# linchaobao/EPPM

Measured on AMD Instinct MI355X. Metric: Mflow-vectors/sec, higher is better.
Workload: dtype f32; 1 GPU; single 1024x436 Sintel-shape synthetic pair per step, full 3-level pyramid, patch_r=9, default defs.h parameters; 1 rank(s), independent pairs; inputs: RGBA planes resident in HBM before the timed region; outputs: interleaved float2 flow left in HBM (the PCIe-inclusive window of the reference API -- host RGB in, host u/v out -- is `host_boundary`, with --full); inputs=device-resident RGBA, outputs=device-resident float2 flow, pairs_in_flight_per_gpu=24, pairs_per_launch=8, contexts_in_flight=3, width=1024, height=436

## Files before the change

eppm_amd/_lib.py:

```python
import ctypes as C
import os

from .build import lib_path


class EppmError(RuntimeError):
    pass


class CParams(C.Structure):
    _fields_ = [("patch_r", C.c_int), ("num_iter", C.c_int), ("search_range", C.c_int), ("num_guess", C.c_int),
                ("seg_len", C.c_int), ("wmf_iters", C.c_int), ("seed", C.c_ulonglong), ("propagation", C.c_int),
                ("levels", C.c_int)]


class CTrackParams(C.Structure):
    _fields_ = [("spacing", C.c_int), ("min_eig", C.c_int64), ("fb_alpha", C.c_float), ("fb_beta", C.c_float), ("mb_alpha", C.c_float),
                ("mb_beta", C.c_float), ("capacity", C.c_int)]


class CTFilterParams(C.Structure):
    _fields_ = [("thresh", C.c_float), ("n_max", C.c_int)]


# ... 50 lines not shown

    def as_dict(self):
        return {k: int(getattr(self, k)) for k, _ in self._fields_}


class CObject(C.Structure):
    _fields_ = [("id", C.c_int32), ("age", C.c_int32), ("area", C.c_int32), ("x0", C.c_int32), ("y0", C.c_int32), ("x1", C.c_int32),
                ("y1", C.c_int32), ("n_flow", C.c_int32), ("sum_x", C.c_int64), ("sum_y", C.c_int64), ("sum_qu", C.c_int64), ("sum_qv", C.c_int64)]

    def as_dict(self):
        return {k: int(getattr(self, k)) for k, _ in self._fields_}


class CObjectsCounts(C.Structure):
    _fields_ = [("n", C.c_int32), ("n_found", C.c_int32), ("n_components", C.c_int32), ("next_id", C.c_int32)]

    def as_dict(self):
        return {k: int(getattr(self, k)) for k, _ in self._fields_}


class CTrackCounts(C.Structure):
    _fields_ = [("live", C.c_int), ("ended", C.c_int), ("seeded", C.c_int), ("dropped", C.c_int), ("frame", C.c_int), ("next_id", C.c_int)]

    def as_dict(self):
        return {k: int(getattr(self, k)) for k, _ in self._fields_}


_lib = None

SYMBOLS = [
    "eppm_default_params", "eppm_create", "eppm_create_batch", "eppm_batch_size", "eppm_batch_set_images", "eppm_batch_set_images_device",
    "eppm_batch_compute", "eppm_batch_compute_device", "eppm_batch_compute_end", "eppm_batch_get_plane", "eppm_destroy", "eppm_set_stream", "eppm_set_images", "eppm_set_images_device",
    "eppm_compute", "eppm_compute_begin", "eppm_compute_end", "eppm_compute_device", "eppm_synchronize", "eppm_num_levels", "eppm_level_dims", "eppm_get_plane",
    "eppm_stage_times", "eppm_clear_stage_times", "eppm_enable_stage_timing", "eppm_last_error", "eppm_version",
    "eppm_device_count", "eppm_set_device", "eppm_malloc_device", "eppm_malloc_pitched", "eppm_free_device",
    "eppm_memcpy_h2d", "eppm_memcpy_d2h", "eppm_memcpy2d_h2d", "eppm_memcpy2d_d2h", "eppm_memset_device",
    "eppm_device_synchronize", "eppm_device_mem_info", "eppm_device_pci_bus_id", "eppm_bind_thread_to_device", "eppm_release_cached_memory", "eppm_set_launcher_stream", "eppm_set_launcher_params", "eppm_launcher_status",
    "baoCudaPatchMatchMultiscalePrepare", "baoCudaCensusTransform", "baoCudaPatchMatch", "baoCudaLeftRightCheck",
    "baoCudaOutlierRemoval", "baoCudaWeightedMedianFilter", "baoCudaFillHole", "baoCudaNNF2Flow", "baoCudaBLF_C2F",
    "baoCudaBLFCostFilterRefine", "baoCudaFlowSmoothing", "eppm_flow_to_color", "eppm_compute_color",
    "eppm_pm_rng_create", "eppm_pm_rng_reset", "eppm_pm_rng_destroy", "eppm_pm_rng_block_states", "eppm_pm_gen_rand_field",
    "eppm_pm_cost_field", "eppm_pm_seg_propagate", "eppm_pm_jump_propagate", "eppm_pm_parallel_propagate", "eppm_pm_random_search", "eppm_gauss_filter_rgba", "eppm_resize_rgba",
    "eppm_resize_flow",
    "eppm_host_register", "eppm_host_unregister", "eppm_host_is_registered", "eppm_host_alloc", "eppm_host_free",
    "eppm_compute_begin_into", "eppm_batch_compute_begin_into",
    "eppm_load_ppm", "eppm_ppm_size", "eppm_save_flo", "eppm_load_flo", "eppm_flo_size", "eppm_flow_error",
    "eppm_flow_error_border", "eppm_flow_error_percentage", "eppm_flow_cutoff", "eppm_flow_to_color_host",
    "eppm_compute_bidirectional", "eppm_compute_bidirectional_device", "eppm_batch_compute_bidirectional", "eppm_set_occlusion_params",
    "eppm_fb_occlusion", "eppm_fb_occlusion_host",
    "eppm_interpolate", "eppm_interpolate_device", "eppm_batch_interpolate", "eppm_interpolate_frames", "eppm_interpolate_host",
    "eppm_track_default_params", "eppm_track_capacity", "eppm_tracker_create", "eppm_tracker_destroy", "eppm_track_step",
    "eppm_track_step_frames", "eppm_tracker_get", "eppm_tracker_get_ended", "eppm_tracker_set", "eppm_track_step_host", "eppm_track_seeds_host",
    "eppm_push_image", "eppm_push_image_device", "eppm_set_temporal", "eppm_temporal_reset", "eppm_temporal_valid", "eppm_temporal_prior_host",
    "eppm_temporal_prior",
    "eppm_batch_set_temporal", "eppm_batch_push_images", "eppm_batch_push_images_device", "eppm_batch_temporal_valid", "eppm_batch_temporal_reset",
    "eppm_temporal_prior_batch",
    "eppm_set_stop_level", "eppm_stop_level", "eppm_flow_upsample",
    "eppm_tfilter_default_params", "eppm_tfilter_create", "eppm_tfilter_create_size", "eppm_tfilter_destroy", "eppm_tfilter_reset", "eppm_tfilter_step",
    "eppm_tfilter_step_frames", "eppm_tfilter_get", "eppm_tfilter_get_device", "eppm_tfilter_get_state", "eppm_tfilter_set_state",
    "eppm_tfilter_seed_host", "eppm_tfilter_step_host",
    "eppm_stab_default_params", "eppm_stab_create", "eppm_stab_create_size", "eppm_stab_destroy", "eppm_stab_reset", "eppm_stab_step",
    "eppm_stab_step_frames", "eppm_stab_get", "eppm_stab_get_device", "eppm_stab_get_mask", "eppm_stab_get_model", "eppm_stab_get_path",
    "eppm_stab_set_path", "eppm_gmotion_fit_host", "eppm_stab_update_host", "eppm_stab_warp_host",
    "eppm_cutdet_default_params", "eppm_cutdet_create", "eppm_cutdet_create_size", "eppm_cutdet_destroy", "eppm_cutdet_step",
    "eppm_cutdet_step_frames", "eppm_cutdet_get", "eppm_cutdet_cuts", "eppm_cutdet_host",
    "eppm_mblur_default_params", "eppm_motion_blur", "eppm_motion_blur_device", "eppm_batch_motion_blur", "eppm_motion_blur_frames",
    "eppm_motion_blur_host",
    "eppm_cmap_default_params", "eppm_cmap_create", "eppm_cmap_create_size", "eppm_cmap_destroy", "eppm_cmap_reset", "eppm_cmap_step",
    "eppm_cmap_step_frames", "eppm_cmap_get_state", "eppm_cmap_set_state", "eppm_cmap_set_layer", "eppm_cmap_render", "eppm_cmap_render_device",
    "eppm_cmap_age", "eppm_cmap_step_host", "eppm_cmap_render_host",
    "eppm_objects_default_params", "eppm_objects_create", "eppm_objects_create_size", "eppm_objects_destroy", "eppm_objects_reset",
    "eppm_objects_step", "eppm_objects_step_frames", "eppm_objects_get", "eppm_objects_get_labels", "eppm_objects_get_state",
    "eppm_objects_set_state", "eppm_objects_label_host", "eppm_objects_carry_host", "eppm_objects_assign_host",
    "eppm_plate_default_params", "eppm_plate_create", "eppm_plate_create_size", "eppm_plate_destroy", "eppm_plate_reset", "eppm_plate_canvas_dims",
    "eppm_plate_step", "eppm_plate_step_frames", "eppm_plate_render", "eppm_plate_render_frames", "eppm_plate_get", "eppm_plate_get_device",
    "eppm_plate_get_mask", "eppm_plate_get_path", "eppm_plate_set_path", "eppm_plate_get_state", "eppm_plate_set_state",
    "eppm_plate_forms_host", "eppm_plate_block_host", "eppm_plate_accumulate_host", "eppm_plate_render_host",
    "eppm_defect_default_params", "eppm_defect_create", "eppm_defect_create_size", "eppm_defect_destroy", "eppm_defect_reset", "eppm_defect_step",
    "eppm_defect_step_frames", "eppm_defect_get", "eppm_defect_get_device", "eppm_defect_get_mask", "eppm_defect_get_stats",
    "eppm_defect_get_state", "eppm_defect_set_state", "eppm_defect_step_host",
]


TEST_SYMBOLS = ["eppm_test_set_option", "eppm_test_c2f_refine_batch", "eppm_probe_c2f_window", "eppm_probe_dispatch", "eppm_probe_fast_exp", "eppm_probe_div_const", "eppm_probe_delta_table",
                "eppm_probe_unpack_texel", "eppm_probe_pm_parity", "eppm_probe_ctx_rng_states", "eppm_test_pm_search", "eppm_probe_search_pretest", "eppm_probe_launch_log"]

_variant = None


def select_library(variant):
    global _variant
    if _lib is not None and variant != _variant:
        raise EppmError("select_library: a library is loaded already")
    _variant = variant


def lib():
    global _lib
    if _lib is None:
        path = lib_path(_variant)
        if not os.path.exists(path):
            raise EppmError(f"{path} is missing: run eppm_amd.build() (hipcc --offload-arch=gfx950); there is no CPU fallback")
        L = C.CDLL(path)
        L.eppm_last_error.restype = C.c_char_p
        L.eppm_version.restype = C.c_char_p
        _plate_signatures(L)
        _lib = L
    return _lib


def _plate_signatures(L):
    P, I, Z, F = C.c_void_p, C.c_int, C.c_size_t, C.c_float
    sig = {
        "eppm_plate_default_params": [P], "eppm_plate_create": [P, P, P], "eppm_plate_create_size": [I, I, I, I, P, P], "eppm_plate_destroy": [P],
        "eppm_plate_reset": [P, I], "eppm_plate_canvas_dims": [P, P, P], "eppm_plate_step": [P, P, P],
        "eppm_plate_step_frames": [P, I, P, Z, P, P, I], "eppm_plate_render": [P, P, I, P, Z, P],
        "eppm_plate_render_frames": [P, I, P, Z, P, P, P, Z, P], "eppm_plate_get": [P, I, P, Z, P], "eppm_plate_get_device": [P, I, P, Z],
        "eppm_plate_get_mask": [P, I, P], "eppm_plate_get_path": [P, I, P], "eppm_plate_set_path": [P, I, P], "eppm_plate_get_state": [P, I, P],
        "eppm_plate_set_state": [P, I, P], "eppm_plate_forms_host": [P, P, P, P], "eppm_plate_block_host": [P, P, I, I, P],
        "eppm_plate_accumulate_host": [P, P, P, P, I, I, P], "eppm_plate_render_host": [P, P, I, P, P, I, I, P, P, P],
    }
    for name, args in sig.items():
        fn = getattr(L, name, None)
        if fn is None:
            continue
        fn.argtypes = args
        fn.restype = I


def check(status, what=""):
    if status != 0:
        raise EppmError(f"{what}: status {status}: {lib().eppm_last_error().decode()}")


def check_launcher(what=""):
    check(lib().eppm_launcher_status(), what)


LAUNCH_STAGES = ("smoothing", "jbu", "refine", "search", "sweep", "sweeps_merged")


class launch_log:

    def __enter__(self):
        check(lib().eppm_test_set_option(b"launch_log", 1), "launch_log on")
        self._kept = None
        return self

    def entries(self):
        if self._kept is not None:
            return self._kept
        n = lib().eppm_probe_launch_log(None, 0)
        buf = (C.c_int * (6 * max(n, 1)))()
        n = min(n, lib().eppm_probe_launch_log(buf, n))
        return [(LAUNCH_STAGES[buf[6 * i]],) + tuple(buf[6 * i + 1:6 * i + 6]) for i in range(n)]

    def __exit__(self, *exc):
        self._kept = self.entries()
        lib().eppm_test_set_option(b"launch_log", 0)
        return False


def probe_dispatch(stage, *args, nout=1):
    a = (C.c_int * len(args))(*[int(v) for v in args])
    out = (C.c_int * nout)()
    check(lib().eppm_probe_dispatch(stage.encode(), a, len(args), out, nout), f"eppm_probe_dispatch {stage}")
    return tuple(out)
# ... 1 lines not shown
```

eppm_amd/csrc/api_internal.h:

```cpp
#pragma once

#include <ctype.h>
#include <math.h>
#include <sched.h>
#include <stdarg.h>
#include <stdio.h>
#include <stdlib.h>
#include <string.h>

#include <atomic>
#include <chrono>
#include <condition_variable>
#include <map>
#include <mutex>
#include <string>
#include <tuple>
#include <vector>

#include "eppm_internal.h"
#include "host_registry.h"

#define EPPM_HIDDEN __attribute__((visibility("hidden")))

EPPM_HIDDEN int set_err(int code, const char* fmt, ...) __attribute__((format(printf, 2, 3)));
#define HIPCHK(expr)                                                                                         \
    do {                                                                                                     \
        hipError_t e_ = (expr);                                                                              \
        if (e_ != hipSuccess) {                                                                              \
            (void)hipGetLastError();                                                                         \
            return set_err(EPPM_ERR_HIP, "%s failed: %s (%s:%d)", #expr, hipGetErrorString(e_), __FILE__, __LINE__); \
        }                                                                                                    \
    } while (0)
#define CHK(expr)                     \
    do {                              \
        int r_ = (expr);              \
        if (r_ != EPPM_OK) return r_; \
    } while (0)

EPPM_HIDDEN int check_params(const eppm_params& p);
EPPM_HIDDEN void host_pm_lut(int R, std::vector<float>& v);
EPPM_HIDDEN void host_wmf_lut(std::vector<float>& v);
EPPM_HIDDEN void host_blf_lut(std::vector<float>& v);
EPPM_HIDDEN int pyr_init_dim(int* arrH, int* arrW, int h, int w, int maxDepth, double ratio);
EPPM_HIDDEN int upload_lut(float** dst, const std::vector<float>& v);
struct DeltaIndex { int32_t t1[256]; std::vector<float> dval; };
EPPM_HIDDEN const DeltaIndex& delta_index();
EPPM_HIDDEN int upload_lut_delta(float** dst, const std::vector<float>& head, int which);
EPPM_HIDDEN int upload_pm_lut(float** dst, int R);
EPPM_HIDDEN int upload_wmf_lut(float** dst);
EPPM_HIDDEN int upload_blf_lut(float** dst);

#ifdef EPPM_TEST_HOOKS
EPPM_HIDDEN extern std::atomic<int> g_opt_rand_table;
EPPM_HIDDEN extern std::atomic<int> g_opt_sweep_spec;
EPPM_HIDDEN extern std::atomic<int> g_opt_no_split;
EPPM_HIDDEN extern std::atomic<int> g_opt_force_split;
EPPM_HIDDEN extern std::atomic<int> g_opt_search_pre;
static inline int opt_rand_table() { return g_opt_rand_table.load(); }
static inline int opt_sweep_spec() { return g_opt_sweep_spec.load(); }
static inline int opt_no_split() { return g_opt_no_split.load(); }
static inline int opt_force_split() { return g_opt_force_split.load(); }
static inline int opt_search_pre() { return g_opt_search_pre.load(); }
EPPM_HIDDEN extern std::atomic<int> g_opt_alloc_fill;
static inline int opt_alloc_fill() { return g_opt_alloc_fill.load(); }
EPPM_HIDDEN hipError_t alloc_fill(hipError_t e, void* p, size_t bytes, bool pinned);
#else
static constexpr int opt_rand_table() { return 1; }
static constexpr int opt_sweep_spec() { return -1; }
static constexpr int opt_no_split() { return 0; }
static constexpr int opt_force_split() { return 0; }
static constexpr int opt_search_pre() { return -1; }
static constexpr int opt_alloc_fill() { return -1; }
#endif


namespace eppm { struct RngTables; }
struct eppm_pm_rng {
    eppm::RngTables* tables = nullptr;
    const int16_t* rand_tab = nullptr;
    size_t rand_stride = 0;
    int device = 0, w = 0, h = 0, gx = 0, gy = 0, G = 0, per_lane = 0;
    unsigned long long seed = 0;
    uint32_t* init_tab = nullptr;
    uint32_t* iter_tab = nullptr;
    uint32_t* work[2][2] = {{nullptr, nullptr}, {nullptr, nullptr}};
    bool own_work = true;
    int cur[2] = {0, 0};
    uint32_t* skip_mat = nullptr;
    uint32_t skip_weyl = 0;
    eppm::PmRngDev dev() const
    {
        eppm::PmRngDev d;
        d.init_tab = init_tab; d.iter_tab = iter_tab; d.skip_mat = skip_mat;
        d.skip_weyl = skip_weyl; d.per_lane = per_lane; d.gx = gx; d.gy = gy;
        return d;
    }
};
EPPM_HIDDEN int rng_create(eppm_pm_rng** out, int w, int h, const eppm_params& p, bool alloc_work = true);
EPPM_HIDDEN void rng_free(eppm_pm_rng* r);
EPPM_HIDDEN void rngtab_release_idle();

EPPM_HIDDEN hipError_t cache_alloc(void** p, size_t bytes, bool pinned, int device);
EPPM_HIDDEN void cache_free(void* p, size_t bytes, bool pinned, int device);
EPPM_HIDDEN hipError_t pooled_stream_create(hipStream_t* out, int device);
EPPM_HIDDEN void pooled_stream_destroy(hipStream_t s, int device);

EPPM_HIDDEN eppm::PmProblem mk_problem(const eppm::PlanesH& P, float* cost, int16_t* nnf, int16_t* nnf_alt, eppm_pm_rng* rng, int k, float* spec = nullptr,
                                       int32_t* scand = nullptr, uint32_t* wl = nullptr, int16_t* seed = nullptr, float* restw = nullptr);
EPPM_HIDDEN void search(eppm::PmBatch& b, eppm_pm_rng* rng, const float* lut, const eppm_params& prm, hipStream_t s, int launch_no = -1, bool pretest = false);
EPPM_HIDDEN bool sweep_list_on(int mode);
EPPM_DECISION bool sweep_speculative(int iteration, long long pixels, int m);
EPPM_DECISION bool sweeps_merged(int iteration, long long pixels, long long problem_pixels, int m);
EPPM_HIDDEN void sweep(eppm::PmBatch& b, const float* lut, const eppm_params& prm, int dir, hipStream_t s, bool speculative = false);
EPPM_HIDDEN void jump(eppm::PmBatch& b, const float* lut, const eppm_params& prm, hipStream_t s);
EPPM_HIDDEN void neighbor(eppm::PmBatch& b, const float* lut, const eppm_params& prm, int launches, hipStream_t s);
EPPM_HIDDEN void run_patchmatch(eppm::PmBatch& b, eppm_pm_rng* rng, const float* lut, const eppm_params& prm, hipStream_t s, int spec_mode, int pre_from = -1);
EPPM_HIDDEN void pm_start(eppm::PmBatch& b, eppm_pm_rng* rng, const float* lut, const eppm_params& prm, hipStream_t s, int pre_from = -1);
EPPM_HIDDEN void pm_iterate(eppm::PmBatch& b, eppm_pm_rng* rng, const float* lut, const eppm_params& prm, hipStream_t s, int spec_mode, int pre_from = -1);
#ifndef EPPM_SWEEP_CACHE
#define EPPM_SWEEP_CACHE 1
#endif

EPPM_HIDDEN int launcher_finish();

EPPM_HIDDEN int ctx_device(const eppm_ctx* c, int* h, int* w);
EPPM_HIDDEN void ctx_stage_begin(eppm_ctx* c, const char* name);
EPPM_HIDDEN void ctx_stage_end(eppm_ctx* c);

EPPM_HIDDEN int stab_step_on(eppm_stab* f, eppm::StabArgs& in, int slot0, const uint8_t* cut, hipStream_t s, eppm_ctx* timing);
EPPM_HIDDEN const uint8_t* stab_mask_device(const eppm_stab* f, size_t* slot_stride);
EPPM_HIDDEN const char* stab_model_device(const eppm_stab* f, size_t* slot_stride);
```

eppm_amd/csrc/c2f_device.cuh:

```cuda
#pragma once
#include "eppm_device.cuh"

#ifndef EPPM_C2F_UNROLL
#define EPPM_C2F_UNROLL 2
#endif
#ifndef EPPM_C2F_WAVES
#define EPPM_C2F_WAVES 4
#endif
#ifndef EPPM_C2F_WAVES_MIN
#define EPPM_C2F_WAVES_MIN 2
#endif
#define EPPM_C2F_OCC __attribute__((amdgpu_waves_per_eu(EPPM_C2F_WAVES_MIN, EPPM_C2F_WAVES)))
#ifndef EPPM_C2F_WIN_H
#ifdef EPPM_TOL
#define EPPM_C2F_WIN_H 50
#else
#define EPPM_C2F_WIN_H 48
#endif
#endif
#ifndef EPPM_C2F_PASS2
#define EPPM_C2F_PASS2 1
#endif
#ifndef EPPM_C2F_WIN_WAVES
#define EPPM_C2F_WIN_WAVES 4
#endif
#ifndef EPPM_C2F_SPLIT_BELOW_WAVES
#define EPPM_C2F_SPLIT_BELOW_WAVES 1024
#endif
#ifndef EPPM_C2F_WINDOW
#define EPPM_C2F_WINDOW 1
#endif
#ifndef EPPM_C2F_WINDOW17
#define EPPM_C2F_WINDOW17 1
#endif
#ifdef EPPM_TOL
#define EPPM_C2F_LOG2 true
#else
#define EPPM_C2F_LOG2 false
#endif
#define EPPM_PRAGMA_(x) _Pragma(#x)
#define EPPM_UNROLL(n) EPPM_PRAGMA_(unroll n)

namespace eppm {

__device__ __forceinline__ Planes to_dev(const PlanesH& h, size_t pstride = 0, unsigned pair = 0)
{
    Planes p;
    p.pk1 = pair_ptr((const float4*)h.pk1, pstride, pair); p.pk2 = pair_ptr((const float4*)h.pk2, pstride, pair);
    p.w = h.w; p.h = h.h; p.pitch = h.pitch;
    return p;
}

__device__ __forceinline__ float4 stage_texel(const uint32_t* __restrict__ pc, const float4* __restrict__ pk, unsigned idx)
{
    if (pc) { const uint32_t w = pc[idx]; return make_texel(w, w >> 24); }
    return pk[idx];
}

__device__ __forceinline__ bool c2f_unknown(float fvx, float fvy) { return fvx > kUnknownFlowThresh || fvy > kUnknownFlowThresh; }
__device__ __forceinline__ int c2f_centre(float f, int x) { return (int)(int16_t)(f2short(f) + x); }
__device__ __forceinline__ void c2f_store_flow(float* flow, int idx, int fx, int fy)
{
    flow[idx * 2] = (float)fx;
    flow[idx * 2 + 1] = (float)fy;
}
__device__ __forceinline__ float c2f_min(float a, float b) { return (a < b) ? a : b; }
__device__ __forceinline__ float c2f_min4(float c1, float c2, float c3, float c4) { return c2f_min(c1, c2f_min(c2, c2f_min(c3, c4))); }
template <class F>
__device__ __forceinline__ void c2f_select_best(float* flow, int x, int y, int ccx, int ccy, int w, int h, F cost_of)
{
    int bx = ccx, by = ccy;
    float min_cost = 999999;
#pragma unroll
    for (int m = 0; m < 3; m++) {
        const int cx = (int)(int16_t)(ccx + m - 1);
        if (cx < 0 || cx >= w) continue;
#pragma unroll
        for (int n = 0; n < 3; n++) {
            const int cy = (int)(int16_t)(ccy + n - 1);
            if (cy < 0 || cy >= h) continue;
            const float cv = cost_of(m, n);
            if (cv < min_cost) { min_cost = cv; bx = cx; by = cy; }
        }
    }
    flow[(y * w + x) * 2] = (float)(bx - x);
    flow[(y * w + x) * 2 + 1] = (float)(by - y);
}

template <int SPLIT>
__device__ __forceinline__ bool c2f_tile_origin(const Planes& P, int& x0, int& y0, int& part)
{
    const int tiles_x = (P.w + kBlock - 1) / kBlock, tiles = tiles_x * ((P.h + kBlock - 1) / kBlock);
    const int per_xcd = (tiles + 7) / 8;
    const int slot = SPLIT ? (blockIdx.x >> 3) / SPLIT : (blockIdx.x >> 3);
    part = SPLIT ? (blockIdx.x >> 3) % SPLIT : -1;
    const int tile = (blockIdx.x & 7) * per_xcd + slot;
    if (slot >= per_xcd || tile >= tiles) return false;
    x0 = (tile % tiles_x) * kBlock; y0 = (tile / tiles_x) * kBlock;
    return true;
}

template <int R> struct C2fSrcTile { static constexpr int TWU = kBlock + 2 * R, TW = (TWU + 15) / 16 * 16; };
struct C2fOff { int dx16, up; };

template <int R>
struct C2fTables {
    static constexpr int S = R + 1;
    C2fOff off[3][S * S];
    int rowdy[3][S];
};

constexpr int cfloor(float v) { const int t = (int)v; return ((float)t > v) ? t - 1 : t; }
template <int R>
constexpr C2fTables<R> make_c2f_tables()
{
    constexpr int S = R + 1;
    constexpr float kc[3][4] = {
        {0.177f, -0.011f, -0.003f, 0.301f},
        {0.125f, -0.357f, 0.009f, 0.308f},
        {0.205f, 0.370f, 0.011f, 0.296f},
    };
    C2fTables<R> T{};
    for (int p = 0; p < 3; p++)
        for (int ii = 0; ii < S; ii++) {
            const int i = 2 * ii - R;
            int dy[S] = {};
            int lo = 1 << 30;
            for (int jj = 0; jj < S; jj++) {
                const int j = 2 * jj - R;
                const float fx = (float)(j)*kc[p][0] + (float)(i)*kc[p][1];
                const float fy = (float)(j)*kc[p][2] + (float)(i)*kc[p][3];
                T.off[p][ii * S + jj].dx16 = (j + cfloor(fx)) * 16;
                dy[jj] = i + cfloor(fy);
                lo = dy[jj] < lo ? dy[jj] : lo;
            }
            T.rowdy[p][ii] = lo;
            for (int jj = 0; jj < S; jj++) T.off[p][ii * S + jj].up = dy[jj] - lo;
        }
    return T;
}
template <int R> __device__ __forceinline__ const C2fTables<R>& c2f_tables();

template <int R>
struct C2fWinShape {
    static constexpr int xlo() { int v = -R; const auto T = make_c2f_tables<R>(); for (int p = 0; p < 3; p++) for (int t = 0; t < (R + 1) * (R + 1); t++) v = T.off[p][t].dx16 / 16 < v ? T.off[p][t].dx16 / 16 : v; return v; }
    static constexpr int xhi() { int v = R; const auto T = make_c2f_tables<R>(); for (int p = 0; p < 3; p++) for (int t = 0; t < (R + 1) * (R + 1); t++) v = T.off[p][t].dx16 / 16 > v ? T.off[p][t].dx16 / 16 : v; return v; }
    static constexpr int ylo() { int v = -R; const auto T = make_c2f_tables<R>(); for (int p = 0; p < 3; p++) for (int i = 0; i <= R; i++) v = T.rowdy[p][i] < v ? T.rowdy[p][i] : v; return v; }
    static constexpr int yhi() { int v = R; const auto T = make_c2f_tables<R>(); for (int p = 0; p < 3; p++) for (int i = 0; i <= R; i++) v = T.rowdy[p][i] + 1 > v ? T.rowdy[p][i] + 1 : v; return v; }
    static constexpr int XLO = xlo(), XHI = xhi(), YLO = ylo(), YHI = yhi();
    static constexpr int WW = (R == 9) ? 64 : (kBlock + 2 + (XHI - XLO) + 8 + 15) / 16 * 16;
    static constexpr int WH = (R == 9) ? EPPM_C2F_WIN_H : kBlock + 2 + (YHI - YLO) + 7;
    static constexpr int SPAN_X = WW - 3 - (XHI - XLO), SPAN_Y = WH - 3 - (YHI - YLO);
    static_assert(SPAN_X >= kBlock - 1 && SPAN_Y >= kBlock - 1, "window too small for a constant-flow tile (spread kBlock - 1)");
};

#ifdef EPPM_TOL
struct C2fSample { rgbf p1; uint32_t k1; float lsrc; };
__device__ __forceinline__ rgbf c2f_weight_centre(const rgbf c) { return tol_scale_centre(c); }
template <class LUT>
__device__ __forceinline__ C2fSample c2f_sample(const LUT& L, const rgbf c1, const float4 q1, int t)
{
    const rgbf p1 = texel_rgb(q1);
    const uint32_t k1 = __float_as_uint(q1.w);
    return {p1, k1, tol_exp_arg_scaled(c1, p1, L.gsp[t])};
}
template <class LUT>
__device__ __forceinline__ void c2f_term(const LUT& L, const C2fSample& s, const rgbf c2, const float4 q2, float& cs, float& ws)
{
    const rgbf p2 = texel_rgb(q2);
    const float cost = tol_cost(L.tab(), s.p1, p2, s.k1, __float_as_uint(q2.w));
    patch_accum(cs, ws, cost, __builtin_amdgcn_exp2f(tol_exp_arg_scaled(c2, p2, s.lsrc)));
}
#else
struct C2fSample { rgbf p1; uint32_t k1; float a2, gsp; };
__device__ __forceinline__ rgbf c2f_weight_centre(const rgbf c) { return c; }
template <class LUT>
__device__ __forceinline__ C2fSample c2f_sample(const LUT& L, const rgbf c1, const float4 q1, int t)
{
    const rgbf p1 = texel_rgb(q1);
    const uint32_t k1 = __float_as_uint(q1.w);
    float a2 = max_abs_diff(c1, p1);
    a2 *= a2;
    return {p1, k1, a2, L.gsp[t]};
}
template <class LUT>
// ... 71 lines not shown
template <int R, int PASS, bool RAW = false, bool WIN = false, int WW = 0>
__device__ __forceinline__ void c2f_pass(const Planes& P, const PatchLutT<R + 1>& L, const float4* __restrict__ s_src,
                                         int TW, int tx, int ty, int cx16, int wmax16, int ccy, const rgbf c1, const rgbf (&c2)[3], float (&run)[3],
                                         const float4* __restrict__ s_win = nullptr, int wbase = 0)
{
    constexpr int S = R + 1;
    constexpr int TP = (PASS == 0) ? 0 : PASS - 1;
    const C2fTables<R>& T = c2f_tables<R>();
    const rgbf c1w = c2f_weight_centre(c1), c2w[3] = {c2f_weight_centre(c2[0]), c2f_weight_centre(c2[1]), c2f_weight_centre(c2[2])};
    float cs[3] = {0.0f, 0.0f, 0.0f}, ws[3] = {0.0f, 0.0f, 0.0f};
    const unsigned pitch16 = (unsigned)P.pitch << 4;
#pragma unroll 1
    for (int ii = 0; ii < S; ii++) {
        unsigned Rr[4];
        const int rdy = (PASS == 0) ? 2 * ii - R : T.rowdy[TP][ii];
        const int rb = ccy - 1 + rdy;
        if (!WIN) {
#pragma unroll
            for (int k = 0; k < 4; k++) Rr[k] = __umul24((unsigned)iclamp(rb + k, 0, P.h - 1), pitch16);
        }
EPPM_UNROLL(EPPM_C2F_UNROLL)
        for (int jj = 0; jj < S; jj++) {
            const C2fSample smp = c2f_sample(L, c1w, s_src[(ty + 2 * ii) * TW + tx + 2 * jj], ii * S + jj);
            const int dx16 = (PASS == 0) ? (2 * jj - R) * 16 : T.off[TP][ii * S + jj].dx16;
            float4 q2[3];
            if (WIN) {
                const int soff = (rdy + ((PASS != 0) ? T.off[TP][ii * S + jj].up : 0)) * (WW * 16) + dx16;
                const char* wp = reinterpret_cast<const char*>(s_win) + (wbase + soff);
#pragma unroll
                for (int n = 0; n < 3; n++) q2[n] = *reinterpret_cast<const float4*>(wp + n * (WW * 16));
            } else {
                const unsigned Xb = (unsigned)med3i(cx16 + dx16, 0, wmax16);
                if (PASS != 0 && T.off[TP][ii * S + jj].up) {
#pragma unroll
                    for (int n = 0; n < 3; n++) q2[n] = texel_at(P.pk2, Rr[n + 1] + Xb);
                } else {
#pragma unroll
                    for (int n = 0; n < 3; n++) q2[n] = texel_at(P.pk2, Rr[n] + Xb);
                }
            }
#pragma unroll
            for (int n = 0; n < 3; n++) c2f_term(L, smp, c2w[n], q2[n], cs[n], ws[n]);
        }
    }
#pragma unroll
    for (int n = 0; n < 3; n++) {
        const float c = cs[n] / ws[n];
        run[n] = (RAW || PASS == 3) ? c : c2f_min(c, run[n]);
    }
}

template <int R, int PA, int PB, int WW>
__device__ __forceinline__ void c2f_pass2_win(const PatchLutT<R + 1>& L, const float4* __restrict__ s_src, int TW, int tx, int ty,
                                              const rgbf c1, const rgbf (&c2)[3], const float4* __restrict__ s_win, int wbase,
                                              float (&outA)[3], float (&outB)[3])
{
    constexpr int S = R + 1;
    constexpr int TA = (PA == 0) ? 0 : PA - 1, TB = (PB == 0) ? 0 : PB - 1;
    const C2fTables<R>& T = c2f_tables<R>();
    const rgbf c1w = c2f_weight_centre(c1), c2w[3] = {c2f_weight_centre(c2[0]), c2f_weight_centre(c2[1]), c2f_weight_centre(c2[2])};
    const rgbf c2w6[6] = {c2w[0], c2w[1], c2w[2], c2w[0], c2w[1], c2w[2]};
    float cs[6] = {0.0f, 0.0f, 0.0f, 0.0f, 0.0f, 0.0f}, ws[6] = {0.0f, 0.0f, 0.0f, 0.0f, 0.0f, 0.0f};
#pragma unroll 1
    for (int ii = 0; ii < S; ii++) {
        const int rdyA = (PA == 0) ? 2 * ii - R : T.rowdy[TA][ii];
        const int rdyB = (PB == 0) ? 2 * ii - R : T.rowdy[TB][ii];
EPPM_UNROLL(EPPM_C2F_UNROLL)
        for (int jj = 0; jj < S; jj++) {
            const C2fSample smp = c2f_sample(L, c1w, s_src[(ty + 2 * ii) * TW + tx + 2 * jj], ii * S + jj);
            const int soffA = (rdyA + ((PA != 0) ? T.off[TA][ii * S + jj].up : 0)) * (WW * 16) + ((PA == 0) ? (2 * jj - R) * 16 : T.off[TA][ii * S + jj].dx16);
            const int soffB = (rdyB + ((PB != 0) ? T.off[TB][ii * S + jj].up : 0)) * (WW * 16) + ((PB == 0) ? (2 * jj - R) * 16 : T.off[TB][ii * S + jj].dx16);
            const char* wa = reinterpret_cast<const char*>(s_win) + (wbase + soffA);
            const char* wb = reinterpret_cast<const char*>(s_win) + (wbase + soffB);
            float4 q[6];
#pragma unroll
            for (int n = 0; n < 3; n++) { q[n] = *reinterpret_cast<const float4*>(wa + n * (WW * 16)); q[3 + n] = *reinterpret_cast<const float4*>(wb + n * (WW * 16)); }
            c2f_terms<6>(L, smp, c2w6, q, cs, ws);
        }
    }
#pragma unroll
    for (int n = 0; n < 3; n++) { outA[n] = cs[n] / ws[n]; outB[n] = cs[3 + n] / ws[3 + n]; }
}

}
```

eppm_amd/csrc/context.cpp:

```cpp
#include "context.h"

using namespace eppm;

extern "C" int eppm_destroy(eppm_ctx* c)
{
    if (!c) return EPPM_OK;
    (void)hipSetDevice(c->device);
    if (c->stream) (void)hipStreamSynchronize(c->stream);
    c->out_hold.release();
    clear_events(c, c->ev);
    clear_events(c, c->ev_prep);
    for (hipEvent_t e : c->ev_pool) (void)hipEventDestroy(e);
    cache_free(c->slab, c->slab_bytes, false, c->device);
    if (c->h_color) (void)hipHostFree(c->h_color);
    for (int q = 0; q < 2; q++) {
        cache_free(c->h_rgb[q], c->h_rgb_bytes, true, c->device);
        if (c->ev_rgb[q]) (void)hipEventDestroy(c->ev_rgb[q]);
    }
    if (c->ev_h2d) (void)hipEventDestroy(c->ev_h2d);
    cache_free(c->h_flow, c->h_flow_bytes, true, c->device);
    cache_free(c->bwd, c->bwd_bytes, false, c->device);
    cache_free(c->h_bwd, c->h_bwd_bytes, true, c->device);
    cache_free(c->itp, c->itp_bytes, false, c->device);
    cache_free(c->h_itp, c->h_itp_bytes, true, c->device);
// ... 11 lines not shown
    struct Entry { int device, R; float *pm, *wmf, *blf; };
    static std::mutex mu;
    static std::vector<Entry> tab;
    std::lock_guard<std::mutex> lk(mu);
    for (const Entry& e : tab)
        if (e.device == device && e.R == R) { *pm = e.pm; *wmf = e.wmf; *blf = e.blf; return EPPM_OK; }
    Entry e{device, R, nullptr, nullptr, nullptr};
    CHK(upload_pm_lut(&e.pm, R));
    CHK(upload_wmf_lut(&e.wmf));
    CHK(upload_blf_lut(&e.blf));
    tab.push_back(e);
    *pm = e.pm; *wmf = e.wmf; *blf = e.blf;
    return EPPM_OK;
}

static int ctx_alloc(eppm_ctx* c)
{
    const int h = c->h, w = c->w;
    Carve cv;
    auto pitch_of = [](size_t row_bytes) { return (row_bytes + 255) & ~(size_t)255; };
    c->raw_pitch = pitch_of((size_t)w * 4);
    for (uint32_t** p : {&c->raw1, &c->raw2}) cv.plane(p, c->raw_pitch * h);
    for (int i = 0; i < c->nl; i++) {
        c->ipitch[i] = pitch_of((size_t)c->W[i] * 4);
        c->cpitch[i] = pitch_of((size_t)c->W[i]);
        const size_t n = (size_t)c->W[i] * c->H[i];
        for (uint32_t** p : {&c->img1[i], &c->img2[i], &c->tmpu[i]}) cv.plane(p, c->ipitch[i] * c->H[i]);
        for (void** p : {&c->pk1[i], &c->pk2[i]}) cv.plane(p, n * 16);
        for (uint32_t** p : {&c->pc1[i], &c->pc2[i]}) cv.plane(p, n * 4);
        for (uint8_t** p : {&c->cen1[i], &c->cen2[i]}) cv.plane(p, c->cpitch[i] * c->H[i]);
        for (float** p : {&c->flow[i], &c->flow_tmp[i]}) cv.plane(p, n * 8);
        if (i < c->nl - 1 && c2f_refine_wants_split(c->W[i], c->H[i], c->prm.patch_r, 1, c->opt_no_split != 0)) cv.plane(&c->c2f_cost9[i], n * 36 * 4);
    }
    const int L = c->nl - 1;
    const size_t n2 = (size_t)c->W[L] * c->H[L];
#ifndef EPPM_TOL
    if (c->prm.patch_r == 9)
#endif
    {
        c->pp_pad = (c->prm.patch_r + 2) & ~1;
        c->pp_pitch = parity_pitch(c->W[L], c->pp_pad);
        for (uint32_t** p : {&c->pp1, &c->pp2}) cv.plane(p, (size_t)2 * c->H[L] * c->pp_pitch * 4);
    }
    for (int16_t** p : {&c->nnf1, &c->nnf2, &c->nnf_tmp, &c->nnf_tmp2}) cv.plane(p, n2 * 4);
    for (float** p : {&c->cost1, &c->cost2}) cv.plane(p, n2 * 4);
    for (float** p : {&c->spec1, &c->spec2}) cv.plane(p, n2 * 4 * 4);
    if (pm_search_pretest_form(c->W[L], c->H[L], c->prm.patch_r, 2, c->npairs))
        for (float** p : {&c->restw1, &c->restw2}) cv.plane(p, n2 * 4);
    for (int32_t** p : {&c->scand1, &c->scand2}) cv.plane(p, n2 * 4 * 4);
    for (uint32_t** p : {&c->wl1, &c->wl2}) cv.plane(p, pm_worklist_words(c->W[L], c->H[L], c->prm.seg_len) * 4);
    for (int16_t** p : {&c->seed1, &c->seed2}) cv.plane(p, n2 * 4 * 4);
    cv.plane(&c->wmf_ws, wmf_workspace_words(c->W[L], c->H[L], c->prm.wmf_iters) * 4);
    cv.plane(&c->d_rgb, (size_t)h * w * 3 * 2);
    cv.plane(&c->d_color, (size_t)h * w * 4);
    cv.plane(&c->d_uv, (size_t)h * w * 8);
    CHK(rng_create(&c->rng, c->W[L], c->H[L], c->prm, false));
    const size_t rng_bytes = (size_t)c->rng->gx * c->rng->gy * 64 * 6 * 4;
    for (int k = 0; k < 2; k++)
        for (int q = 0; q < 2; q++) cv.plane(&c->rng->work[k][q], rng_bytes);
    c->stride = (cv.off + 4095) & ~(size_t)4095;
    CHK(cv.alloc(&c->slab, &c->slab_bytes, c->stride * c->npairs, c->device, (std::to_string(c->npairs) + " slab(s)").c_str()));
    CHK(shared_luts(c->device, c->prm.patch_r, &c->lut_pm, &c->lut_wmf, &c->lut_blf));
    c->out_u.assign(c->npairs, nullptr);
    c->out_v.assign(c->npairs, nullptr);
    for (auto* v : {&c->tmp_snap, &c->tmp_valid, &c->tmp_seeded, &c->tmp_cut}) v->assign(c->npairs, 0);
    return EPPM_OK;
}

extern "C" int eppm_create_batch(eppm_ctx** out, int h, int w, int device, const eppm_params* params, int npairs)
{
    if (!out) return set_err(EPPM_ERR_ARG, "eppm_create: NULL out");
    *out = nullptr;
    if (npairs < 1 || npairs > 4096) return set_err(EPPM_ERR_ARG, "eppm_create_batch: npairs %d out of range [1,4096]", npairs);
    if (h < 4 || w < 4 || h > 32767 || w > 32767) return set_err(EPPM_ERR_ARG, "eppm_create: size %dx%d out of range (NNF coordinates are int16)", w, h);
    if ((unsigned long long)h * (unsigned long long)w * 16ULL >= (1ULL << 32))
        return set_err(EPPM_ERR_ARG, "eppm_create: size %dx%d out of range (texel planes are addressed with 32-bit byte offsets)", w, h);
    eppm_params p;
    eppm_default_params(&p);
    if (params) p = *params;
    CHK(check_params(p));
    HIPCHK(hipSetDevice(device));
    eppm_ctx* c = new eppm_ctx();
    c->device = device; c->prm = p; c->h = h; c->w = w; c->npairs = npairs; c->n_active = 1;
    c->opt_sweep_spec = opt_sweep_spec(); c->opt_no_split = opt_no_split(); c->opt_search_pre = opt_search_pre();
    c->nl = pyr_init_dim(c->H, c->W, h, w, p.levels, 0.5f);
    const int L = c->nl - 1;
    if (c->H[L] < 1 || c->W[L] < 1 || (c->W[L] + p.seg_len - 1) / p.seg_len > 1024 || (c->H[L] + p.seg_len - 1) / p.seg_len > 1024) {
        delete c;
        return set_err(EPPM_ERR_ARG, "eppm_create: unsupported size %dx%d", w, h);
    }
    const hipError_t e = pooled_stream_create(&c->stream, c->device);
    if (e != hipSuccess) { delete c; return set_err(EPPM_ERR_HIP, "hipStreamCreate: %s", hipGetErrorString(e)); }
    c->own_stream = true;
    int r = ctx_alloc(c);
    if (r != EPPM_OK) { eppm_destroy(c); return r; }
    *out = c;
    return EPPM_OK;
}

extern "C" int eppm_create(eppm_ctx** out, int h, int w, int device, const eppm_params* params)
{
    return eppm_create_batch(out, h, w, device, params, 1);
}

extern "C" int eppm_batch_size(const eppm_ctx* c) { return c ? c->npairs : 0; }

extern "C" int eppm_set_stream(eppm_ctx* c, void* s)
{
    if (!c) return set_err(EPPM_ERR_ARG, "NULL ctx");
    if (c->own_stream && c->stream) { (void)hipStreamSynchronize(c->stream); pooled_stream_destroy(c->stream, c->device); }
    c->stream = (hipStream_t)s;
    c->own_stream = false;
    return EPPM_OK;
}

extern "C" int eppm_num_levels(const eppm_ctx* c) { return c ? c->nl : 0; }
extern "C" int eppm_level_dims(const eppm_ctx* c, int level, int* h, int* w)
{
    if (!c || level < 0 || level >= c->nl) return set_err(EPPM_ERR_ARG, "bad level");
    if (h) *h = c->H[level];
    if (w) *w = c->W[level];
    return EPPM_OK;
}
extern "C" int eppm_enable_stage_timing(eppm_ctx* c, int on)
{
    if (!c) return set_err(EPPM_ERR_ARG, "NULL ctx");
    c->timing = (on == 2) ? 2 : (on != 0);
    return EPPM_OK;
}

int ctx_device(const eppm_ctx* c, int* h, int* w)
{
    *h = c->h;
    *w = c->w;
    return c->device;
}

void ctx_stage_begin(eppm_ctx* c, const char* name) { stage_begin(c, c->ev, name); }
void ctx_stage_end(eppm_ctx* c) { stage_end(c, c->ev); }

extern "C" int eppm_synchronize(eppm_ctx* c)
{
    if (!c) return set_err(EPPM_ERR_ARG, "NULL ctx");
    HIPCHK(hipStreamSynchronize(c->stream));
    return EPPM_OK;
}

extern "C" int eppm_stage_times(eppm_ctx* c, const char** names, float* ms, int max)
{
    if (!c) return 0;
    (void)hipStreamSynchronize(c->stream);
    int n = 0;
    for (auto* v : {&c->ev_prep, &c->ev})
        for (auto& e : *v) {
            if (n >= max) return n;
            float t = 0;
            if (hipEventElapsedTime(&t, e.a, e.b) != hipSuccess) t = -1;
            names[n] = e.name; ms[n] = t; n++;
        }
    return n;
}

extern "C" int eppm_clear_stage_times(eppm_ctx* c)
{
    if (!c) return set_err(EPPM_ERR_ARG, "NULL ctx");
    (void)hipStreamSynchronize(c->stream);
    clear_events(c, c->ev);
// ... 86 lines not shown
```

eppm_amd/csrc/context.h:

```cpp
#pragma once

#include <algorithm>

#include "api_internal.h"

struct StageEv { const char* name; hipEvent_t a, b; };

struct eppm_ctx {
    int device = 0;
    hipStream_t stream = nullptr;
    bool own_stream = false;
    int opt_sweep_spec = -1, opt_no_split = 0, opt_search_pre = -1;
    eppm_params prm;
    int h = 0, w = 0, nl = 0;
    int stop_level = 0;
    int npairs = 1, n_active = 1;
    char* slab = nullptr;
    size_t stride = 0;
    int H[eppm::kMaxLevels], W[eppm::kMaxLevels];
    size_t ipitch[eppm::kMaxLevels], cpitch[eppm::kMaxLevels];
    uint32_t *raw1 = nullptr, *raw2 = nullptr;
    size_t raw_pitch = 0;
    uint32_t *img1[eppm::kMaxLevels] = {}, *img2[eppm::kMaxLevels] = {}, *tmpu[eppm::kMaxLevels] = {};
    uint8_t *cen1[eppm::kMaxLevels] = {}, *cen2[eppm::kMaxLevels] = {};
    void *pk1[eppm::kMaxLevels] = {}, *pk2[eppm::kMaxLevels] = {};
    uint32_t *pc1[eppm::kMaxLevels] = {}, *pc2[eppm::kMaxLevels] = {};
    uint32_t *pp1 = nullptr, *pp2 = nullptr;
    int pp_pitch = 0, pp_pad = 0;
    int16_t *nnf1 = nullptr, *nnf2 = nullptr, *nnf_tmp = nullptr, *nnf_tmp2 = nullptr;
    float *cost1 = nullptr, *cost2 = nullptr;
    float *spec1 = nullptr, *spec2 = nullptr;
    int32_t *scand1 = nullptr, *scand2 = nullptr;
    uint32_t *wl1 = nullptr, *wl2 = nullptr;
    float *restw1 = nullptr, *restw2 = nullptr;
    int16_t *seed1 = nullptr, *seed2 = nullptr;
    uint32_t* wmf_ws = nullptr;
    bool flow_pending = false;
    float *flow[eppm::kMaxLevels] = {}, *flow_tmp[eppm::kMaxLevels] = {};
    float* c2f_cost9[eppm::kMaxLevels] = {};
    float *lut_pm = nullptr, *lut_wmf = nullptr, *lut_blf = nullptr;
    eppm_pm_rng* rng = nullptr;
    float* d_uv = nullptr;
    uint32_t* d_color = nullptr;
    uint32_t* h_color = nullptr;
    uint8_t* d_rgb = nullptr;
    size_t slab_bytes = 0, h_rgb_bytes = 0, h_flow_bytes = 0;
    uint8_t* h_rgb[2] = {nullptr, nullptr};
    hipEvent_t ev_rgb[2] = {nullptr, nullptr};
    hipEvent_t ev_h2d = nullptr;
    int rgb_cur = 0;
    float* h_flow = nullptr;
    std::vector<float*> out_u, out_v;
    eppm::HostHold out_hold;
    bool have_images = false, have_flow = false;
    char* bwd = nullptr;
    size_t bwd_stride = 0, bwd_bytes = 0, h_bwd_bytes = 0;
    float* bflow[eppm::kMaxLevels] = {};
    float* d_buv = nullptr;
    uint8_t *occ1 = nullptr, *occ2 = nullptr;
    uint8_t* h_bwd = nullptr;
    float occ_alpha = 0.01f, occ_beta = 0.5f;
    bool have_bwd = false;
    bool bwd_images = false;
    char* itp = nullptr;
    size_t itp_bytes = 0, itp_plane = 0, h_itp_bytes = 0;
    uint64_t* itp_keys = nullptr;
    int32_t *itp_fill1 = nullptr, *itp_fill2 = nullptr;
    uint8_t* itp_rgb = nullptr;
    uint8_t* h_itp = nullptr;
    char* mbl = nullptr;
    size_t mbl_bytes = 0, mbl_plane = 0, mbl_tplane = 0, h_mbl_bytes = 0;
    uint32_t* mbl_packed = nullptr;
    uint64_t* mbl_tkeys = nullptr;
    uint8_t* mbl_rgb = nullptr;
    uint8_t* h_mbl = nullptr;
    bool temporal = false;
    std::vector<uint8_t> tmp_snap;
    std::vector<uint8_t> tmp_valid;
    std::vector<uint8_t> tmp_seeded;
    std::vector<uint8_t> tmp_cut;
    char* tmp = nullptr;
    size_t tmp_bytes = 0, tmp_stride = 0;
    int16_t *prev_fwd = nullptr, *prev_bwd = nullptr, *prior1 = nullptr, *prior2 = nullptr, *nnf_init1 = nullptr, *nnf_init2 = nullptr;
    float *cost_init1 = nullptr, *cost_init2 = nullptr;
    int32_t* tmp_keys = nullptr;
    void tmp_drop() { std::fill(tmp_valid.begin(), tmp_valid.end(), 0); std::fill(tmp_snap.begin(), tmp_snap.end(), 0); std::fill(tmp_cut.begin(), tmp_cut.end(), 0); }
    int timing = 0;
    std::vector<StageEv> ev;
    std::vector<StageEv> ev_prep;
    std::vector<hipEvent_t> ev_pool;
    eppm::Batch bt() const { return eppm::Batch{n_active, stride}; }
    template <class T> T* of_pair(T* p, int k) const { return (T*)((char*)p + (size_t)k * stride); }
    template <class T> T* of_bwd_pair(T* p, int k) const { return (T*)((char*)p + (size_t)k * bwd_stride); }
};

// ... 83 lines not shown
```

eppm_amd/csrc/ctx_compute.cpp:

```cpp
#include "context.h"
#include "temporal.h"

using namespace eppm;

static int tmp_alloc(eppm_ctx* c)
{
    if (c->tmp) return EPPM_OK;
    const int L = c->nl - 1;
    const size_t n2 = (size_t)c->W[L] * c->H[L];
    Carve cv;
    for (int16_t** p : {&c->prev_fwd, &c->prev_bwd, &c->prior1, &c->prior2, &c->nnf_init1, &c->nnf_init2}) cv.plane(p, n2 * 4);
    for (float** p : {&c->cost_init1, &c->cost_init2}) cv.plane(p, n2 * 4);
    cv.plane(&c->tmp_keys, n2 * 4 * 2);
    c->tmp_stride = cv.off;
    CHK(cv.alloc(&c->tmp, &c->tmp_bytes, c->tmp_stride * c->npairs, c->device, "temporal planes"));
    for (int k = 0; k < c->npairs; k++) launch_temporal_keys_init((int32_t*)((char*)c->tmp_keys + (size_t)k * c->tmp_stride), (int)(2 * n2), c->stream);
    HIPCHK(hipGetLastError());
    return EPPM_OK;
}

static int set_temporal(eppm_ctx* c, int on)
{
    c->temporal = on != 0;
    if (!on) c->tmp_drop();
// ... 7 lines not shown
}
extern "C" int eppm_temporal_reset(eppm_ctx* c)
{
    if (!c) return set_err(EPPM_ERR_ARG, "eppm_temporal_reset: NULL ctx");
    return eppm_batch_temporal_reset(c, 0);
}
extern "C" int eppm_temporal_valid(const eppm_ctx* c) { return eppm_batch_temporal_valid(c, 0); }

extern "C" int eppm_batch_set_temporal(eppm_ctx* c, int on)
{
    if (!c) return set_err(EPPM_ERR_ARG, "eppm_batch_set_temporal: NULL ctx");
    return set_temporal(c, on);
}
extern "C" int eppm_batch_temporal_reset(eppm_ctx* c, int pair)
{
    if (!c) return set_err(EPPM_ERR_ARG, "eppm_batch_temporal_reset: NULL ctx");
    if (pair >= c->npairs) return set_err(EPPM_ERR_ARG, "eppm_batch_temporal_reset: pair %d, context holds %d", pair, c->npairs);
    for (int k = pair < 0 ? 0 : pair; k < (pair < 0 ? c->npairs : pair + 1); k++) c->tmp_valid[k] = c->tmp_snap[k] = 0;
    return EPPM_OK;
}
extern "C" int eppm_batch_temporal_valid(const eppm_ctx* c, int pair)
{
    return c && pair >= 0 && pair < c->npairs && c->temporal && c->tmp_valid[pair] ? 1 : 0;
}

struct Branch {
    int16_t *&nnf, *&nnf_alt;
    float* cost;
    uint32_t* const* guide;
    bool swap, bwd, dominant;
    int16_t* snapshot;
    float *a[kMaxLevels], *b[kMaxLevels];
};

enum { kStageUp, kStageRefine, kStageBlf, kStageJbu };
static const struct EPPM_HIDDEN LevelStageNames {
    char s[4][2][kMaxLevels][24];
    LevelStageNames()
    {
        const char* base[4] = {"upsample", "c2f_refine", "flow_blf", "flow_jbu"};
        for (int k = 0; k < 4; k++)
            for (int b = 0; b < 2; b++)
                for (int l = 0; l < kMaxLevels; l++) snprintf(s[k][b][l], sizeof s[k][b][l], "%s%s_L%d", base[k], b ? "_bwd" : "", l);
    }
} level_stage;

static void branch_nnf2flow(eppm_ctx* c, Branch& d)
{
    hipStream_t s = c->stream;
    const Batch bt = c->bt();
    const int L = c->nl - 1, lw = c->W[L], lh = c->H[L], gp = (int)(c->ipitch[L] / 4);
    launch_outlier(d.nnf_alt, d.cost, d.nnf, lw, lh, lw, lw, s, bt);
    std::swap(d.nnf, d.nnf_alt);
    if (launch_wmf(d.nnf, d.nnf_alt, d.guide[L], gp, lw, lh, lw, c->lut_wmf, c->prm.wmf_iters, 1, c->wmf_ws, s, bt) != d.nnf)
        std::swap(d.nnf, d.nnf_alt);
    launch_fill_holes(d.nnf_alt, d.nnf, d.guide[L], gp, lw, lh, lw, s, bt);
    std::swap(d.nnf, d.nnf_alt);
    if (d.snapshot) launch_nnf2flow_snapshot(d.a[L], lw, d.snapshot, c->tmp_stride, d.nnf, lw, lw, lh, s, bt);
    else launch_nnf2flow(d.a[L], lw, d.nnf, lw, lw, lh, s, bt);
}

static int branch_c2f(eppm_ctx* c, Branch& d, int (*keep)(eppm_ctx*, int, float*))
{
    hipStream_t s = c->stream;
    const Batch bt = c->bt();
    const int L = c->nl - 1;
    auto blf = [&](float* dst, const float* src, int l) { launch_flow_blf(dst, src, d.guide[l], (int)(c->ipitch[l] / 4), c->W[l], c->H[l], c->W[l], c->lut_blf, s, bt); };
    const int stop = c->stop_level;
    float* r = d.a[L];
    for (int l = L - 1; l >= 0; l--) {
        if (l < stop) {
            stage_begin(c, c->ev, level_stage.s[kStageJbu][d.bwd][l]);
            float* out = (r == d.b[l]) ? d.a[l] : d.b[l];
            launch_flow_jbu(out, r, d.guide[l], (int)(c->ipitch[l] / 4), c->W[l], c->H[l], c->W[l + 1], c->H[l + 1], c->lut_blf, s, bt);
            r = out;
            CHK(keep(c, l, r));
            stage_end(c, c->ev);
            continue;
        }
        stage_begin(c, c->ev, level_stage.s[kStageUp][d.bwd][l]);
        launch_resize_flow(d.a[l], c->H[l], c->W[l], r, c->H[l + 1], c->W[l + 1], 2.0f, 2.0f, s, bt);
        stage_end(c, c->ev);
        stage_begin(c, c->ev, level_stage.s[kStageRefine][d.bwd][l], d.dominant);
        launch_c2f_refine(planes(c, l, d.swap), d.a[l], c->lut_pm, c->prm.patch_r, c->c2f_cost9[l], s, bt, c->opt_no_split != 0);
        stage_end(c, c->ev, d.dominant);
        stage_begin(c, c->ev, level_stage.s[kStageBlf][d.bwd][l]);
        blf(d.b[l], d.a[l], l);
        r = d.b[l];
        if (l > 0) CHK(keep(c, l, r));
        stage_end(c, c->ev);
    }
    if (stop > 0) return EPPM_OK;
    stage_begin(c, c->ev, d.bwd ? "flow_blf_bwd_final" : "flow_blf_final");
    float* out = (r == d.b[0]) ? d.a[0] : d.b[0];
    blf(out, r, 0);
    CHK(keep(c, 0, out));
    stage_end(c, c->ev);
    return EPPM_OK;
}

static int keep_fwd(eppm_ctx* c, int l, float* r)
{
    if (r != c->flow[l]) std::swap(c->flow[l], c->flow_tmp[l]);
    return EPPM_OK;
}

static int compute_all(eppm_ctx* c)
{
    if (!c->have_images) return set_err(EPPM_ERR_STATE, "eppm_compute: no images set");
    HIPCHK(hipSetDevice(c->device));
    c->have_bwd = false;
    hipStream_t s = c->stream;
    const Batch bt = c->bt();
    const int L = c->nl - 1, lw = c->W[L], lh = c->H[L];

    const bool tmode = c->temporal;
    bool seeded = false;
    std::fill(c->tmp_seeded.begin(), c->tmp_seeded.end(), 0);
    if (tmode) {
        CHK(tmp_alloc(c));
        TemporalArgs a{};
        for (int k = 0; k < bt.n; k++)
            if (c->tmp_valid[k]) { a.armed[k >> 5] |= 1u << (k & 31); seeded = true; }
        if (seeded) {
            a.prev[0] = c->prev_fwd; a.prior[0] = c->prior1; a.keys[0] = c->tmp_keys; a.step[0] = 1;
            a.prev[1] = c->prev_bwd; a.prior[1] = c->prior2; a.keys[1] = c->tmp_keys + (size_t)lw * lh; a.step[1] = -1;
            a.w = lw; a.h = lh; a.ndir = 2; a.nslots = bt.n; a.stride = c->tmp_stride;
            stage_begin(c, c->ev, "temporal_advect");
            launch_temporal_splat(a, s);
            launch_temporal_gather(a, s);
            stage_end(c, c->ev);
        }
    }
    std::fill(c->tmp_snap.begin(), c->tmp_snap.end(), 0);

    const size_t pm_entry = c->ev.size();
    stage_begin(c, c->ev, "patchmatch");
    {
        PmBatch b;
        b.n = 2; b.cpitch = lw; b.npitch = lw; b.npairs = bt.n; b.stride = bt.stride;
        b.cache_plane = (size_t)lw * lh;
        b.seed_plane = (size_t)lw * lh * 2;
        b.wl_units = pm_worklist_units(lw, lh, c->prm.seg_len);
        b.p[0] = mk_problem(planes(c, L, false), c->cost1, c->nnf1, c->nnf_tmp, c->rng, 0, c->spec1, EPPM_SWEEP_CACHE ? c->scand1 : nullptr, sweep_list_on(c->opt_sweep_spec) ? c->wl1 : nullptr, c->seed1, c->restw1);
        b.p[1] = mk_problem(planes(c, L, true), c->cost2, c->nnf2, c->nnf_tmp2, c->rng, 1, c->spec2, EPPM_SWEEP_CACHE ? c->scand2 : nullptr, sweep_list_on(c->opt_sweep_spec) ? c->wl2 : nullptr, c->seed2, c->restw2);
        if (!seeded) run_patchmatch(b, c->rng, c->lut_pm, c->prm, s, c->opt_sweep_spec, c->opt_search_pre);
        else {
            pm_start(b, c->rng, c->lut_pm, c->prm, s, c->opt_search_pre);
            PmSeed sd;
            sd.prior[0] = c->prior1; sd.nnf_init[0] = c->nnf_init1; sd.cost_init[0] = c->cost_init1;
            sd.prior[1] = c->prior2; sd.nnf_init[1] = c->nnf_init2; sd.cost_init[1] = c->cost_init2;
            sd.stride = c->tmp_stride;
            stage_begin(c, c->ev, "temporal_select");
            launch_pm_cost_select(b, sd, c->lut_pm, c->prm.patch_r, s);
            stage_end(c, c->ev);
            pm_iterate(b, c->rng, c->lut_pm, c->prm, s, c->opt_sweep_spec, c->opt_search_pre);
        }
    }
    stage_end_at(c, c->ev, pm_entry);
    if (tmode) launch_temporal_snapshot(c->prev_bwd, c->tmp_stride, c->nnf2, lw, lw, lh, s, bt);

    stage_begin(c, c->ev, "l2_post");
    launch_lr_check(c->nnf1, c->cost1, c->nnf2, lw, lh, lw, lw, s, bt);
    launch_lr_check(c->nnf2, c->cost2, c->nnf1, lw, lh, lw, lw, s, bt);
    Branch d{c->nnf1, c->nnf_tmp, c->cost1, c->img1, false, false, true, tmode ? c->prev_fwd : nullptr};
    for (int l = 0; l <= L; l++) { d.a[l] = c->flow[l]; d.b[l] = c->flow_tmp[l]; }
    branch_nnf2flow(c, d);
// ... 251 lines not shown
```

eppm_amd/csrc/eppm_device.cuh:

```cuda
#pragma once

#include <hip/hip_runtime.h>
#include <stdint.h>
#include <float.h>
#include <type_traits>

#include "eppm_internal.h"

namespace eppm {

template <class T>
__device__ __forceinline__ T* pair_ptr(T* p, size_t stride, unsigned pair)
{
    using Byte = typename std::conditional<std::is_const<T>::value, const char, char>::type;
    return reinterpret_cast<T*>(reinterpret_cast<Byte*>(p) + stride * pair);
}
template <class T>
__device__ __forceinline__ T* pair_ptr_opt(T* p, size_t stride, unsigned pair)
{
    return p ? pair_ptr(p, stride, pair) : p;
}

constexpr float kLambdaAd2 = 0.1f * 0.1f;
constexpr float kPmSigR2 = 0.1f * 0.1f;
// ... 50 lines not shown
    int r;
    asm("v_med3_i32 %0, %1, %2, %3" : "=v"(r) : "v"(v), "v"(lo), "v"(hi));
    return r;
}

__device__ __forceinline__ float max_abs_diff(const rgbf a, const rgbf b)
{
    return fmaxf(fmaxf(fabsf(a.x - b.x), fabsf(a.y - b.y)), fabsf(a.z - b.z));
}

struct Planes {
    const float4* pk1;
    const float4* pk2;
    int w, h;
    int pitch;
};

typedef uint32_t u32x4 __attribute__((ext_vector_type(4)));
typedef uint32_t u32x2 __attribute__((ext_vector_type(2)));

#ifndef EPPM_TOL
#ifndef EPPM_CENSUS_POPCNT
#define EPPM_CENSUS_POPCNT 1
#endif
__device__ __forceinline__ float4 make_texel(uint32_t rgba, uint32_t census)
{
    const rgbf c = unpack_rgb(rgba);
    return make_float4(c.x, c.y, c.z, __uint_as_float(EPPM_CENSUS_POPCNT ? (census & 0xffu) * 0x01010101u : (census & 0xffu) << 2));
}
__device__ __forceinline__ float census_cost(const float* __restrict__ cnx, uint32_t w1, uint32_t w2)
{
    return *reinterpret_cast<const float*>(reinterpret_cast<const char*>(cnx) + (EPPM_CENSUS_POPCNT ? (uint32_t)__builtin_popcount(w1 ^ w2) : (w1 ^ w2)));
}
__device__ __forceinline__ float4 unpack_texel(uint32_t w, uint32_t)
{
    static_assert(EPPM_CENSUS_POPCNT, "the census byte replicated into its word (make_texel)");
    const rgbf c = unpack_rgb(w);
    return make_float4(c.x, c.y, c.z, __uint_as_float(__builtin_amdgcn_perm(w, w, 0x03030303u)));
}
#else
constexpr unsigned kTolScale = 4u;
__device__ __forceinline__ float4 make_texel(uint32_t rgba, uint32_t census)
{
    return make_float4(__uint_as_float((rgba & 0xffu) * kTolScale), __uint_as_float(((rgba >> 8) & 0xffu) * kTolScale),
                       __uint_as_float(((rgba >> 16) & 0xffu) * kTolScale), __uint_as_float((census & 0xffu) * 0x01010101u));
}
#endif
__device__ __forceinline__ float one_minus_fast_exp(float x) { return 1 - fast_exp(x); }

struct DeltaTab {
    int t1[256];
    float t2[kDeltaSlots];
};
#ifndef EPPM_DELTA_PATCH
#define EPPM_DELTA_PATCH 1
#endif
#ifndef EPPM_DELTA_BLF
#define EPPM_DELTA_BLF 1
#endif
typedef const __attribute__((address_space(3))) float lds_cfloat;
typedef const __attribute__((address_space(3))) int lds_cint;
__device__ __forceinline__ uint32_t lds_addr(const void* p) { return (uint32_t)(uintptr_t)(const __attribute__((address_space(3))) void*)p; }
__device__ __forceinline__ uint32_t delta_lookup_l1(const DeltaTab& D, float d)
{
    const uint32_t a1 = __float_as_uint(__builtin_fmaf(d, __uint_as_float(1020u), __uint_as_float(lds_addr(D.t1))));
    return (uint32_t)*reinterpret_cast<lds_cint*>(a1);
}
__device__ __forceinline__ float delta_lookup_l2(float d, uint32_t t1) { return *reinterpret_cast<lds_cfloat*>((__float_as_uint(d) << 2) + t1); }
__device__ __forceinline__ float delta_lookup(const DeltaTab& D, float d) { return delta_lookup_l2(d, delta_lookup_l1(D, d)); }
__device__ __forceinline__ float delta_lookup_off(const DeltaTab& D, float d)
{
    const uint32_t o1 = __float_as_uint(d * __uint_as_float(1020u));
    const uint32_t o2 = (__float_as_uint(d) << 2) + (uint32_t)*reinterpret_cast<const int*>(reinterpret_cast<const char*>(D.t1) + o1);
    return *reinterpret_cast<const float*>(reinterpret_cast<const char*>(D.t2) + o2);
}
template <bool ADDRESSES = true>
__device__ __forceinline__ void load_delta_tab(DeltaTab& D, const float* __restrict__ src, int tid, int nthreads)
{
    const int t2_at = ADDRESSES ? (int)lds_addr(D.t2) : 0;
    for (int t = tid; t < 256; t += nthreads) D.t1[t] = __float_as_int(src[t]) + t2_at;
    for (int t = tid; t < kDeltaSlots; t += nthreads) D.t2[t] = src[256 + t];
}
__device__ __forceinline__ rgbf texel_rgb(const float4 t) { return rgbf{t.x, t.y, t.z}; }

__device__ __forceinline__ float4 tex_px(const float4* img, int pitch, int w, int h, int x, int y)
{
    x = iclamp(x, 0, w - 1);
    y = iclamp(y, 0, h - 1);
    return img[(unsigned)(y * pitch + x)];
}
__device__ __forceinline__ float4 texel_at(const float4* base, unsigned byte_off)
{
    return *reinterpret_cast<const float4*>(reinterpret_cast<const char*>(base) + byte_off);
}
__device__ __forceinline__ unsigned texel_off(int pitch16, int w, int h, int x, int y)
{
    x = iclamp(x, 0, w - 1);
    y = iclamp(y, 0, h - 1);
    return __umul24((unsigned)y, (unsigned)pitch16) + ((unsigned)x << 4);
}
__device__ __forceinline__ unsigned texel_off16(int pitch16, int wmax16, int hmax, int x16, int y)
{
    return __umul24((unsigned)med3i(y, 0, hmax), (unsigned)pitch16) + (unsigned)med3i(x16, 0, wmax16);
}
__device__ __forceinline__ uint32_t tex_rgba(const uint32_t* img, int pitch, int w, int h, int x, int y)
{
    x = iclamp(x, 0, w - 1);
    y = iclamp(y, 0, h - 1);
    return img[(unsigned)(y * pitch + x)];
}

#ifndef EPPM_TOL
struct ExactTables { const float* cnx; const DeltaTab& D; };
__device__ __forceinline__ void patch_terms(const float4 q1, const float4 q2, const rgbf c1, const rgbf c2, float gsp,
                                            const ExactTables T, float& cost_term, float& weight_term)
{
    const float* __restrict__ cnx = T.cnx;
    const DeltaTab& D = T.D;
    const rgbf p1 = texel_rgb(q1);
    const rgbf p2 = texel_rgb(q2);
    float cost = max_abs_diff(p1, p2);
    cost = EPPM_DELTA_PATCH ? delta_lookup(D, cost) : one_minus_fast_exp(div_ad2(-(cost * cost)));
    cost += census_cost(cnx, __float_as_uint(q1.w), __float_as_uint(q2.w));
    float weight = max_abs_diff(c1, p1);
    weight *= weight;
    float temp = max_abs_diff(c2, p2);
    temp *= temp;
    weight = fast_exp(div_ad2(-(weight + temp)));
    weight *= gsp;
    cost *= weight;
    cost_term = cost;
    weight_term = weight;
}
__device__ __forceinline__ void patch_accum(float& cost_sum, float& weight_sum, float cost_term, float weight_term)
{
    cost_sum += cost_term;
    weight_sum += weight_term;
}
#else
struct TolTables {
    float td[256];
    float ta[256];
    float cn[16];
};
__device__ __forceinline__ uint32_t linf_off(const rgbf a, const rgbf b) { return __float_as_uint(max_abs_diff(a, b)); }
__device__ __forceinline__ float tol_at(const float* __restrict__ t, uint32_t byte_off)
{
    return *reinterpret_cast<const float*>(reinterpret_cast<const char*>(t) + byte_off);
}
__device__ __forceinline__ float tol_cost(const TolTables& T, const rgbf p1, const rgbf p2, uint32_t w1, uint32_t w2)
{
    return tol_at(T.td, linf_off(p1, p2)) + tol_at(T.cn, (uint32_t)__builtin_popcount(w1 ^ w2));
}
constexpr float kTolExpC = (float)(1.4426950408889634 / (255.0 * 255.0 * (double)kPmSigR2) / (double)(kTolScale * kTolScale));
constexpr float kTolWeightBias = 24.0f;
__device__ __forceinline__ float tol_exp_arg(uint32_t off4k, float lsrc)
{
    const float kf = __uint_as_float(off4k) * 0x1p100f;
    return __builtin_fmaf(kf * kf, -kTolExpC * 0x1p98f, lsrc);
}
__device__ __forceinline__ rgbf tol_scale_centre(const rgbf c) { return rgbf{c.x * 0x1p100f, c.y * 0x1p100f, c.z * 0x1p100f}; }
__device__ __forceinline__ float tol_exp_arg_scaled(const rgbf cs, const rgbf p, float lsrc)
{
    const float kf = fmaxf(fmaxf(fabsf(__builtin_fmaf(p.x, 0x1p100f, -cs.x)), fabsf(__builtin_fmaf(p.y, 0x1p100f, -cs.y))), fabsf(__builtin_fmaf(p.z, 0x1p100f, -cs.z)));
    return __builtin_fmaf(kf * kf, -kTolExpC * 0x1p98f, lsrc);
}
// ... 196 lines not shown
```

eppm_amd/csrc/eppm_internal.h:

```cpp
#pragma once

#include <hip/hip_runtime.h>
#include <stddef.h>
#include <stdint.h>

#include <atomic>

#include "../../include/eppm.h"

namespace eppm {

constexpr int kMaxLevels = 8;
constexpr int kNumLevels = 3;
constexpr int kBlock = 16;
constexpr int kMaxS = 32;
constexpr int kWmfRadius = 4;
constexpr int kBlfRadius = 10;
constexpr int kDeltaSlots = 800;

struct Batch {
    int n;
    size_t stride;
};
constexpr Batch kOnePair = {1, 0};
// ... 55 lines not shown
    int n;
    int cpitch, npitch;
    int npairs = 1;
    size_t stride = 0;
    size_t cache_plane = 0;
    int wl_units = 0;
    int sweep_seq = 0;
    size_t seed_plane = 0;
    int merged_it = 0;
    int seg_len = 0, nseg_row = 0, nseg_col = 0;
};
int pm_worklist_units(int w, int h, int seg_len);
inline size_t pm_worklist_words(int w, int h, int seg_len) { return 16 + 10 * (size_t)pm_worklist_units(w, h, seg_len); }
struct PmRngDev {
    const uint32_t* init_tab;
    const uint32_t* iter_tab;
    const uint32_t* skip_mat;
    uint32_t skip_weyl;
    int per_lane;
    int gx, gy;
    const int16_t* rand_tab = nullptr;
};
void launch_pm_rand_table(const PmRngDev& rng, uint32_t* work, int16_t* tab, int G, hipStream_t s);
void launch_pm_init_field(const PmBatch& b, const PmRngDev& rng, hipStream_t s);
void launch_pm_cost_field(const PmBatch& b, const float* lut, int R, hipStream_t s);
int pm_parity_kernels(int R);
bool launch_pm_sweep(PmBatch& b, const float* lut, int R, int seg_len, int dir, hipStream_t s, bool speculative = false);
bool launch_pm_sweeps_merged(PmBatch& b, const float* lut, int R, int seg_len, int iteration, hipStream_t s);
void launch_pm_jump(const PmBatch& b, const float* lut, int R, int step, hipStream_t s);
void launch_pm_neighbor(const PmBatch& b, const float* lut, int R, hipStream_t s);
void launch_pm_random_search(const PmBatch& b, const PmRngDev& rng, const float* lut, int R, int search_range, int num_guess,
                             hipStream_t s, bool pretest = false);
void launch_pm_rest_weight(const PmBatch& b, const float* lut, int R, hipStream_t s);
bool pm_search_pretest_ready(const PmBatch& b, const PmRngDev& rng, int R);
struct PmPretestSums { float* n[2]; float* d[2]; };
void launch_pm_pretest_probe(const PmBatch& b, const float* lut, int R, const PmPretestSums& out, hipStream_t s);
EPPM_DECISION bool pm_search_pretest_form(int w, int h, int R, int problems, int npairs);
EPPM_DECISION bool pm_search_pretest(int iteration, int w, int h, int R, int problems, int npairs);
EPPM_DECISION void pm_search_pretest_knobs(int R, int* row0, int* rows, int* from, float* eps);
EPPM_DECISION int pm_search_rows(int w, int h, int R, int problems, int npairs, bool table);
struct SweepForm { int lpc; bool small, pre, tile; };
EPPM_DECISION SweepForm pm_sweep_form(int w, int h, int R, int seg_len, int dir, int problems, int npairs);

struct PmSeed {
    const int16_t* prior[2];
    int16_t* nnf_init[2];
    float* cost_init[2];
    size_t stride = 0;
};
void launch_pm_cost_select(const PmBatch& b, const PmSeed& seed, const float* lut, int R, hipStream_t s);

constexpr int kTemporalMaxSlots = 4096;
struct TemporalArgs {
    const int16_t* prev[2];
    int16_t* prior[2];
    int32_t* keys[2];
    int step[2];
    int w, h, ndir;
    int nslots;
    size_t stride;
    uint32_t armed[kTemporalMaxSlots / 32];
};
void launch_temporal_keys_init(int32_t* keys, int n, hipStream_t s);
void launch_temporal_splat(const TemporalArgs& a, hipStream_t s);
void launch_temporal_gather(const TemporalArgs& a, hipStream_t s);
void launch_temporal_snapshot(int16_t* prev, size_t prev_stride, const int16_t* nnf, int nnf_pitch, int w, int h, hipStream_t s, Batch bt = kOnePair);
void launch_nnf2flow_snapshot(float* flow, int flow_pitch, int16_t* prev, size_t prev_stride, const int16_t* nnf, int nnf_pitch, int w, int h,
                              hipStream_t s, Batch bt = kOnePair);

void launch_lr_check(int16_t* nnf1, float* cost1, const int16_t* nnf2, int w, int h, int cost_pitch, int nnf_pitch, hipStream_t s, Batch bt = kOnePair);
void launch_outlier(int16_t* nnf_out, float* cost, const int16_t* nnf_in, int w, int h, int cost_pitch, int nnf_pitch, hipStream_t s, Batch bt = kOnePair);
size_t wmf_workspace_words(int w, int h, int num_iter);
int16_t* launch_wmf(int16_t* buf_a, int16_t* buf_b, const uint32_t* img, int ipitch, int w, int h, int nnf_pitch,
                    const float* wmf_lut, int num_iter, int only_occlusion, uint32_t* ws, hipStream_t s, Batch bt = kOnePair);
void launch_fill_holes(int16_t* nnf_out, const int16_t* nnf_in, const uint32_t* img, int ipitch, int w, int h, int nnf_pitch,
                       hipStream_t s, Batch bt = kOnePair);
void launch_nnf2flow(float* flow, int flow_pitch, const int16_t* nnf, int nnf_pitch, int w, int h, hipStream_t s, Batch bt = kOnePair);

void launch_resize_flow(float* out, int outH, int outW, const float* in, int h, int w, float ratio, float post_scale, hipStream_t s, Batch bt = kOnePair);
void launch_mul_scalar(float* flow, float scale, int h, int w, hipStream_t s);
EPPM_DECISION int c2f_refine_split_factor(int w, int h, int R, int npairs = 1, bool no_split = false);
bool c2f_refine_wants_split(int w, int h, int R, int npairs = 1, bool no_split = false);
bool c2f_window_span(int R, int* span_x, int* span_y);
void launch_c2f_refine(const PlanesH& P, float* flow, const float* lut, int R, float* cost9, hipStream_t s, Batch bt = kOnePair, bool no_split = false);
void launch_flow_blf(float* out, const float* in, const uint32_t* img, int ipitch, int w, int h, int flow_pitch,
                     const float* blf_lut, hipStream_t s, Batch bt = kOnePair);
EPPM_DECISION int flow_blf_pixels_per_lane(int w, int h, int npairs = 1);
void launch_flow_jbu(float* out, const float* in_coarse, const uint32_t* img, int ipitch, int w, int h, int wc, int hc, const float* blf_lut,
                     hipStream_t s, Batch bt = kOnePair);

void launch_split_flow(float* uv, const float* flow, int n, hipStream_t s, Batch bt = kOnePair);

void launch_fb_occlusion(uint8_t* occ1, uint8_t* occ2, const float* fwd, size_t fwd_stride, const float* bwd, size_t bwd_stride, int h, int w,
                         float alpha, float beta, int npairs, int ndir, hipStream_t s);

constexpr int kInterpChunk = 4;
struct InterpArgs {
    const uint8_t* img1;
    const uint8_t* img2;
    size_t img_pitch, img_stride;
    const float* flow;
    size_t flow_stride;
    const uint8_t* occ1;
    const uint8_t* occ2;
    size_t occ_stride;
    uint64_t* keys;
    int32_t* fill1;
    int32_t* fill2;
    size_t plane;
    uint8_t* rgb;
    uint8_t* rgba[kInterpChunk];
    size_t rgba_pitch;
    int h, w, nt;
    float t[kInterpChunk];
};
void launch_interp_splat(const InterpArgs& a, int npairs, hipStream_t s);
void launch_interp_fill(const InterpArgs& a, int npairs, hipStream_t s);
void launch_interp_blend(const InterpArgs& a, int npairs, hipStream_t s);

struct MBlurArgs {
    const uint8_t* img;
    size_t img_pitch, img_stride;
    const float* flow;
    size_t flow_stride;
    uint32_t* packed;
    uint64_t* tkeys;
    size_t plane, tplane;
    uint8_t* rgb;
    uint8_t* rgba;
    size_t rgba_pitch;
    int h, w, tiles_x, tiles_y;
    float shutter, max_radius;
    int taps;
};
void launch_mblur_pack(const MBlurArgs& a, int npairs, hipStream_t s);
void launch_mblur_gather(const MBlurArgs& a, int npairs, hipStream_t s);

enum {
    kTrackCntLive, kTrackCntNextId, kTrackCntFrame, kTrackCntDropped, kTrackCntEnded, kTrackCntSeeded,
    kTrackCntIdBase, kTrackCntSurv, kTrackCntPrevLive, kTrackCntSeeded0, kTrackCntDropped0, kTrackCntN = 16
};
struct TrackRec;
struct TrackDev {
    struct {
        int spacing;
        long long min_eig;
        float fb_alpha, fb_beta, mb_alpha, mb_beta;
    } p;
    int cap, ncells, ncx;
    float* npos;
    uint8_t* stat;
    TrackRec* ended;
    int32_t* ended_reason;
    uint8_t* cov;
    uint8_t* flags;
    int32_t *blk_s, *blk_e;
    int32_t* blk_c;
    int32_t* cnt;
};
struct TrackIn {
    const uint8_t* img1;
    const uint8_t* img2;
    size_t pitch;
    const float* fwd;
    const float* bwd;
    int h, w;
};
// ... 171 lines not shown
```

eppm_amd/csrc/k_c2f_refine.hip:

```cpp
#include <type_traits>

#include "c2f_device.cuh"
#include "eppm_internal.h"

namespace eppm {

__constant__ C2fTables<9> c2f_tab9 = make_c2f_tables<9>();
__constant__ C2fTables<17> c2f_tab17 = make_c2f_tables<17>();
template <> __device__ __forceinline__ const C2fTables<9>& c2f_tables<9>() { return c2f_tab9; }
template <> __device__ __forceinline__ const C2fTables<17>& c2f_tables<17>() { return c2f_tab17; }

__global__ __launch_bounds__(256) void k_c2f_refine(PlanesH Ph, float* __restrict__ flow_, const float* __restrict__ lut, int R, size_t pstride)
{
    __shared__ EPPM_LUT_ALIGN PatchLut L;
    load_patch_lut(L, lut, R, threadIdx.y * kBlock + threadIdx.x, 256);
    __syncthreads();
    const Planes P = to_dev(Ph, pstride, blockIdx.z);
    float* __restrict__ flow = pair_ptr(flow_, pstride, blockIdx.z);
    const int x = blockIdx.x * kBlock + threadIdx.x, y = blockIdx.y * kBlock + threadIdx.y;
    if (x >= P.w || y >= P.h) return;
    const float fvx = flow[(y * P.w + x) * 2], fvy = flow[(y * P.w + x) * 2 + 1];
    if (c2f_unknown(fvx, fvy)) { c2f_store_flow(flow, y * P.w + x, 0, 0); return; }
    const int ccx = c2f_centre(fvx, x), ccy = c2f_centre(fvy, y);
    int bx = ccx, by = ccy;
// ... 6 lines not shown
            const int cy = (int)(int16_t)(ccy + n - 1);
            if (cx < 0 || cy < 0 || cx >= P.w || cy >= P.h) continue;
            const float cv = patch_dist_planefit(P, L, R, x, y, cx, cy);
            if (cv < min_cost) { min_cost = cv; bx = cx; by = cy; }
        }
    }
    flow[(y * P.w + x) * 2] = (float)(bx - x);
    flow[(y * P.w + x) * 2 + 1] = (float)(by - y);
}

template <int R, int SPLIT>
__global__ __launch_bounds__(256) EPPM_C2F_OCC void k_c2f_refine_tiled(PlanesH Ph, float* __restrict__ flow_, const float* __restrict__ lut,
                                                                       float* __restrict__ cost9_, size_t pstride)
{
    float* __restrict__ flow = pair_ptr(flow_, pstride, blockIdx.y);
    float* __restrict__ cost9 = pair_ptr_opt(cost9_, pstride, blockIdx.y);
    constexpr int TWU = C2fSrcTile<R>::TWU, TW = C2fSrcTile<R>::TW;
    __shared__ EPPM_LUT_ALIGN PatchLutT<R + 1> L;
    __shared__ float4 s_src[TWU * TW];
    const int tid = threadIdx.y * kBlock + threadIdx.x;
    load_patch_lut<EPPM_C2F_LOG2>(L, lut, R, tid, 256);
    const Planes P = to_dev(Ph, pstride, blockIdx.y);
    int x0, y0, part;
    if (!c2f_tile_origin<SPLIT>(P, x0, y0, part)) return;
    const int m_only = (SPLIT == 3) ? part : -1;
    for (int t = tid; t < TWU * TWU; t += 256) {
        const int ry = t / TWU, rx = t % TWU;
        const int sy = iclamp(y0 + ry - R, 0, P.h - 1), sx = iclamp(x0 + rx - R, 0, P.w - 1);
        s_src[ry * TW + rx] = P.pk1[(unsigned)(sy * P.pitch + sx)];
    }
    __syncthreads();
    const int x = x0 + threadIdx.x, y = y0 + threadIdx.y;
    if (x >= P.w || y >= P.h) return;
    const float fvx = flow[(y * P.w + x) * 2], fvy = flow[(y * P.w + x) * 2 + 1];
    if (c2f_unknown(fvx, fvy)) {
        if (SPLIT == 0) c2f_store_flow(flow, y * P.w + x, 0, 0);
        return;
    }
    const int ccx = c2f_centre(fvx, x), ccy = c2f_centre(fvy, y);
    const rgbf c1 = texel_rgb(s_src[(threadIdx.y + R) * TW + threadIdx.x + R]);
    int bx = ccx, by = ccy;
    float min_cost = 999999;
#pragma unroll 1
    for (int m = 0; m < 3; m++) {
        if (SPLIT == 3 && m != m_only) continue;
        const int cx = (int)(int16_t)(ccx + m - 1);
        if (cx < 0 || cx >= P.w) continue;
        rgbf c2[3];
#pragma unroll
        for (int n = 0; n < 3; n++) c2[n] = texel_rgb(tex_px(P.pk2, P.pitch, P.w, P.h, cx, ccy + n - 1));
        float run[3];
        const int cx16 = cx << 4, wmax16 = (P.w - 1) << 4;
        if (SPLIT == 4) {
            if (part == 3) c2f_pass<R, 3, true>(P, L, s_src, TW, threadIdx.x, threadIdx.y, cx16, wmax16, ccy, c1, c2, run);
            else if (part == 2) c2f_pass<R, 2, true>(P, L, s_src, TW, threadIdx.x, threadIdx.y, cx16, wmax16, ccy, c1, c2, run);
            else if (part == 1) c2f_pass<R, 1, true>(P, L, s_src, TW, threadIdx.x, threadIdx.y, cx16, wmax16, ccy, c1, c2, run);
            else c2f_pass<R, 0, true>(P, L, s_src, TW, threadIdx.x, threadIdx.y, cx16, wmax16, ccy, c1, c2, run);
#pragma unroll
            for (int n = 0; n < 3; n++) cost9[(size_t)(y * P.w + x) * 36 + part * 9 + m * 3 + n] = run[n];
            continue;
        }
        c2f_pass<R, 3>(P, L, s_src, TW, threadIdx.x, threadIdx.y, cx16, wmax16, ccy, c1, c2, run);
        c2f_pass<R, 2>(P, L, s_src, TW, threadIdx.x, threadIdx.y, cx16, wmax16, ccy, c1, c2, run);
        c2f_pass<R, 1>(P, L, s_src, TW, threadIdx.x, threadIdx.y, cx16, wmax16, ccy, c1, c2, run);
        c2f_pass<R, 0>(P, L, s_src, TW, threadIdx.x, threadIdx.y, cx16, wmax16, ccy, c1, c2, run);
        if (SPLIT == 3) {
#pragma unroll
            for (int n = 0; n < 3; n++) cost9[(size_t)(y * P.w + x) * 36 + m * 3 + n] = run[n];
            continue;
        }
#pragma unroll
        for (int n = 0; n < 3; n++) {
            const int cy = (int)(int16_t)(ccy + n - 1);
            if (cy < 0 || cy >= P.h) continue;
            const float cv = run[n];
            if (cv < min_cost) { min_cost = cv; bx = cx; by = cy; }
        }
    }
    if (SPLIT != 0) return;
    flow[(y * P.w + x) * 2] = (float)(bx - x);
    flow[(y * P.w + x) * 2 + 1] = (float)(by - y);
}

template <int R>
__global__ __launch_bounds__(512) __attribute__((amdgpu_waves_per_eu(EPPM_C2F_WIN_WAVES, EPPM_C2F_WIN_WAVES)))
void k_c2f_refine_win(PlanesH Ph, float* __restrict__ flow_, const float* __restrict__ lut, size_t pstride)
{
    using W = C2fWinShape<R>;
    constexpr int TWU = C2fSrcTile<R>::TWU, TW = C2fSrcTile<R>::TW, WW = W::WW, WH = W::WH;
    static_assert(TWU * TW * 16 >= 9 * 256 * 4, "the exchange buffer aliases the source tile");
    __shared__ EPPM_LUT_ALIGN PatchLutT<R + 1> L;
    __shared__ float4 s_src[TWU * TW];
    __shared__ float4 s_win[WH * WW];
    __shared__ int s_mm[4];
    float* __restrict__ flow = pair_ptr(flow_, pstride, blockIdx.y);
    const int ptid = threadIdx.y * kBlock + threadIdx.x;
    const int grp = threadIdx.z;
    const int tid = grp * 256 + ptid;
    load_patch_lut<EPPM_C2F_LOG2>(L, lut, R, tid, 512);
    const Planes P = to_dev(Ph, pstride, blockIdx.y);
    const uint32_t* __restrict__ pc1 = pair_ptr_opt(Ph.pc1, pstride, blockIdx.y);
    const uint32_t* __restrict__ pc2 = pair_ptr_opt(Ph.pc2, pstride, blockIdx.y);
    int x0, y0, part;
    if (!c2f_tile_origin<0>(P, x0, y0, part)) return;
    if (tid == 0) { s_mm[0] = 0x7fffffff; s_mm[1] = -0x7fffffff; s_mm[2] = 0x7fffffff; s_mm[3] = -0x7fffffff; }
    for (int t = tid; t < TWU * TWU; t += 512) {
        const int ry = t / TWU, rx = t % TWU;
        const int sy = iclamp(y0 + ry - R, 0, P.h - 1), sx = iclamp(x0 + rx - R, 0, P.w - 1);
        s_src[ry * TW + rx] = stage_texel(pc1, P.pk1, (unsigned)(sy * P.pitch + sx));
    }
    __syncthreads();
    const int x = x0 + threadIdx.x, y = y0 + threadIdx.y;
    const bool inimg = (x < P.w && y < P.h);
    float fvx = 0.0f, fvy = 0.0f;
    if (inimg) { fvx = flow[(y * P.w + x) * 2]; fvy = flow[(y * P.w + x) * 2 + 1]; }
    const bool known = inimg && !(fvx > kUnknownFlowThresh || fvy > kUnknownFlowThresh);
    const int ccx = c2f_centre(fvx, x), ccy = c2f_centre(fvy, y);
    if (known && grp == 0) {
        atomicMin(&s_mm[0], ccx); atomicMax(&s_mm[1], ccx);
        atomicMin(&s_mm[2], ccy); atomicMax(&s_mm[3], ccy);
    }
    __syncthreads();
    const int mnx = s_mm[0], mxx = s_mm[1], mny = s_mm[2], mxy = s_mm[3];
    const bool coherent = (mxx - mnx <= W::SPAN_X) && (mxy - mny <= W::SPAN_Y);
    const int wx0 = mnx - 1 + W::XLO, wy0 = mny - 1 + W::YLO;
    if (coherent && mxx >= mnx) {
        for (int t = tid; t < WH * WW; t += 512) {
            const int sy = iclamp(wy0 + t / WW, 0, P.h - 1), sx = iclamp(wx0 + t % WW, 0, P.w - 1);
            s_win[t] = stage_texel(pc2, P.pk2, (unsigned)(sy * P.pitch + sx));
        }
    }
    __syncthreads();
    float res[9];
    float res1[9];
    if (known) {
        const rgbf c1 = texel_rgb(s_src[(threadIdx.y + R) * TW + threadIdx.x + R]);
#pragma unroll
        for (int m = 0; m < 3; m++) {
            const int cx = (int)(int16_t)(ccx + m - 1);
            float run[3] = {0.0f, 0.0f, 0.0f}, raw[3] = {0.0f, 0.0f, 0.0f};
            if (!(cx < 0 || cx >= P.w)) {
                rgbf c2[3];
                const int cx16 = cx << 4, wmax16 = (P.w - 1) << 4;
                if (coherent) {
                    const int wbase = ((ccy - 1 - wy0) * WW + (cx - wx0)) * 16;
#pragma unroll
                    for (int n = 0; n < 3; n++) c2[n] = texel_rgb(*reinterpret_cast<const float4*>(reinterpret_cast<const char*>(s_win) + wbase + n * (WW * 16)));
#if EPPM_C2F_PASS2
                    if (grp == 0) {
                        float c4[3], c3[3];
                        c2f_pass2_win<R, 3, 2, WW>(L, s_src, TW, threadIdx.x, threadIdx.y, c1, c2, s_win, wbase, c4, c3);
#pragma unroll
                        for (int n = 0; n < 3; n++) run[n] = c2f_min(c3[n], c4[n]);
                    } else {
                        c2f_pass2_win<R, 1, 0, WW>(L, s_src, TW, threadIdx.x, threadIdx.y, c1, c2, s_win, wbase, run, raw);
                    }
#else
                    if (grp == 0) {
                        c2f_pass<R, 3, false, true, WW>(P, L, s_src, TW, threadIdx.x, threadIdx.y, cx16, wmax16, ccy, c1, c2, run, s_win, wbase);
                        c2f_pass<R, 2, false, true, WW>(P, L, s_src, TW, threadIdx.x, threadIdx.y, cx16, wmax16, ccy, c1, c2, run, s_win, wbase);
                    } else {
                        c2f_pass<R, 1, true, true, WW>(P, L, s_src, TW, threadIdx.x, threadIdx.y, cx16, wmax16, ccy, c1, c2, run, s_win, wbase);
                        c2f_pass<R, 0, true, true, WW>(P, L, s_src, TW, threadIdx.x, threadIdx.y, cx16, wmax16, ccy, c1, c2, raw, s_win, wbase);
                    }
#endif
                } else {
#pragma unroll
                    for (int n = 0; n < 3; n++) c2[n] = texel_rgb(tex_px(P.pk2, P.pitch, P.w, P.h, cx, ccy + n - 1));
                    if (grp == 0) {
                        c2f_pass<R, 3>(P, L, s_src, TW, threadIdx.x, threadIdx.y, cx16, wmax16, ccy, c1, c2, run);
                        c2f_pass<R, 2>(P, L, s_src, TW, threadIdx.x, threadIdx.y, cx16, wmax16, ccy, c1, c2, run);
                    } else {
                        c2f_pass<R, 1, true>(P, L, s_src, TW, threadIdx.x, threadIdx.y, cx16, wmax16, ccy, c1, c2, run);
                        c2f_pass<R, 0, true>(P, L, s_src, TW, threadIdx.x, threadIdx.y, cx16, wmax16, ccy, c1, c2, raw);
                    }
                }
            }
#pragma unroll
            for (int n = 0; n < 3; n++) { res[m * 3 + n] = run[n]; res1[m * 3 + n] = raw[n]; }
        }
    }
    __syncthreads();
    float* __restrict__ xch = reinterpret_cast<float*>(s_src);
    if (grp == 0 && known) {
#pragma unroll
        for (int k = 0; k < 9; k++) xch[k * 256 + ptid] = res[k];
    }
    __syncthreads();
    if (grp != 1 || !inimg) return;
    if (!known) { c2f_store_flow(flow, y * P.w + x, 0, 0); return; }
    int bx = ccx, by = ccy;
    float min_cost = 999999;
#pragma unroll
    for (int m = 0; m < 3; m++) {
        const int cx = (int)(int16_t)(ccx + m - 1);
        if (cx < 0 || cx >= P.w) continue;
#pragma unroll
        for (int n = 0; n < 3; n++) {
            const int cy = (int)(int16_t)(ccy + n - 1);
            if (cy < 0 || cy >= P.h) continue;
            const float m34 = xch[(m * 3 + n) * 256 + ptid];
            const float c_2 = res[m * 3 + n], c_1 = res1[m * 3 + n];
            const float cv = c2f_min(c_1, c2f_min(c_2, m34));
            if (cv < min_cost) { min_cost = cv; bx = cx; by = cy; }
        }
    }
    flow[(y * P.w + x) * 2] = (float)(bx - x);
    flow[(y * P.w + x) * 2 + 1] = (float)(by - y);
}

template <int R>
__global__ __launch_bounds__(1024) __attribute__((amdgpu_waves_per_eu(4, 4)))
void k_c2f_refine_win4(PlanesH Ph, float* __restrict__ flow_, const float* __restrict__ lut, size_t pstride)
{
    using W = C2fWinShape<R>;
// ... 52 lines not shown
            if (!(cx < 0 || cx >= P.w)) {
                rgbf c2[3];
                const int cx16 = cx << 4, wmax16 = (P.w - 1) << 4;
                if (coherent) {
                    const int wbase = ((ccy - 1 - wy0) * WW + (cx - wx0)) * 16;
#pragma unroll
                    for (int n = 0; n < 3; n++) c2[n] = texel_rgb(*reinterpret_cast<const float4*>(reinterpret_cast<const char*>(s_win) + wbase + n * (WW * 16)));
                    if (grp == 0) c2f_pass<R, 3, true, true, WW>(P, L, s_src, TW, threadIdx.x, threadIdx.y, cx16, wmax16, ccy, c1, c2, run, s_win, wbase);
                    else if (grp == 1) c2f_pass<R, 2, true, true, WW>(P, L, s_src, TW, threadIdx.x, threadIdx.y, cx16, wmax16, ccy, c1, c2, run, s_win, wbase);
                    else if (grp == 2) c2f_pass<R, 1, true, true, WW>(P, L, s_src, TW, threadIdx.x, threadIdx.y, cx16, wmax16, ccy, c1, c2, run, s_win, wbase);
                    else c2f_pass<R, 0, true, true, WW>(P, L, s_src, TW, threadIdx.x, threadIdx.y, cx16, wmax16, ccy, c1, c2, run, s_win, wbase);
                } else {
#pragma unroll
                    for (int n = 0; n < 3; n++) c2[n] = texel_rgb(tex_px(P.pk2, P.pitch, P.w, P.h, cx, ccy + n - 1));
                    if (grp == 0) c2f_pass<R, 3, true>(P, L, s_src, TW, threadIdx.x, threadIdx.y, cx16, wmax16, ccy, c1, c2, run);
                    else if (grp == 1) c2f_pass<R, 2, true>(P, L, s_src, TW, threadIdx.x, threadIdx.y, cx16, wmax16, ccy, c1, c2, run);
                    else if (grp == 2) c2f_pass<R, 1, true>(P, L, s_src, TW, threadIdx.x, threadIdx.y, cx16, wmax16, ccy, c1, c2, run);
                    else c2f_pass<R, 0, true>(P, L, s_src, TW, threadIdx.x, threadIdx.y, cx16, wmax16, ccy, c1, c2, run);
                }
            }
#pragma unroll
            for (int n = 0; n < 3; n++) res[m * 3 + n] = run[n];
        }
    }
    __syncthreads();
    float* __restrict__ xch = reinterpret_cast<float*>(s_src);
    if (grp != 0 && known) {
#pragma unroll
        for (int k = 0; k < 9; k++) xch[((grp - 1) * 9 + k) * 256 + ptid] = res[k];
    }
    __syncthreads();
    if (grp != 0 || !inimg) return;
    if (!known) { c2f_store_flow(flow, y * P.w + x, 0, 0); return; }
    int bx = ccx, by = ccy;
    float min_cost = 999999;
#pragma unroll
    for (int m = 0; m < 3; m++) {
        const int cx = (int)(int16_t)(ccx + m - 1);
        if (cx < 0 || cx >= P.w) continue;
#pragma unroll
        for (int n = 0; n < 3; n++) {
            const int cy = (int)(int16_t)(ccy + n - 1);
            if (cy < 0 || cy >= P.h) continue;
            const int k = m * 3 + n;
            const float c_4 = res[k], c_3 = xch[k * 256 + ptid], c_2 = xch[(9 + k) * 256 + ptid], c_1 = xch[(18 + k) * 256 + ptid];
            const float cv = c2f_min4(c_1, c_2, c_3, c_4);
            if (cv < min_cost) { min_cost = cv; bx = cx; by = cy; }
        }
    }
    flow[(y * P.w + x) * 2] = (float)(bx - x);
    flow[(y * P.w + x) * 2 + 1] = (float)(by - y);
}

template <int SPLIT>
__global__ __launch_bounds__(256) void k_c2f_select(float* __restrict__ flow_, const float* __restrict__ cost9_, int w, int h, size_t pstride)
{
    float* __restrict__ flow = pair_ptr(flow_, pstride, blockIdx.z);
    const float* __restrict__ cost9 = pair_ptr(cost9_, pstride, blockIdx.z);
    const int x = blockIdx.x * blockDim.x + threadIdx.x, y = blockIdx.y * blockDim.y + threadIdx.y;
    if (x >= w || y >= h) return;
    const float fvx = flow[(y * w + x) * 2], fvy = flow[(y * w + x) * 2 + 1];
    if (c2f_unknown(fvx, fvy)) { c2f_store_flow(flow, y * w + x, 0, 0); return; }
    c2f_select_best(flow, x, y, c2f_centre(fvx, x), c2f_centre(fvy, y), w, h, [=](int m, int n) {
        const float* __restrict__ pc = cost9 + (size_t)(y * w + x) * 36 + m * 3 + n;
        float cv = pc[0];
        if (SPLIT == 4) {
            cv = pc[27];
            cv = c2f_min(pc[18], cv);
            cv = c2f_min(pc[9], cv);
            cv = c2f_min(pc[0], cv);
        }
        return cv;
    });
}

bool c2f_window_span(int R, int* span_x, int* span_y)
{
    if (!(R == 9 || R == 17)) return false;
    *span_x = (R == 9) ? C2fWinShape<9>::SPAN_X : C2fWinShape<17>::SPAN_X;
    *span_y = (R == 9) ? C2fWinShape<9>::SPAN_Y : C2fWinShape<17>::SPAN_Y;
    return true;
}

static bool c2f_table_ok(int w, int h, int R) { return (w + R < 32764) && (h + R < 32764); }

int c2f_refine_split_factor(int w, int h, int R, int npairs, bool no_split)
{
    if (no_split || !(R == 9 || R == 17) || !c2f_table_ok(w, h, R)) return 0;
    const int tiles = ((w + kBlock - 1) / kBlock) * ((h + kBlock - 1) / kBlock);
    if (!(tiles * npairs * 4 < EPPM_C2F_SPLIT_BELOW_WAVES)) return 0;
    auto imbalance = [&](int f) { const int wgs = tiles * f * npairs; return (float)((wgs + 255) / 256) * 256.0f / (float)wgs; };
    return (imbalance(4) < imbalance(3)) ? 4 : 3;
}
bool c2f_refine_wants_split(int w, int h, int R, int npairs, bool no_split) { return c2f_refine_split_factor(w, h, R, npairs, no_split) != 0; }

template <class F>
static void with_radius(int R, F&& f)
{
    if (R == 9) f(std::integral_constant<int, 9>{});
    else f(std::integral_constant<int, 17>{});
}

void launch_c2f_refine(const PlanesH& P, float* flow, const float* lut, int R, float* cost9, hipStream_t s, Batch bt, bool no_split)
{
    dim3 grid((P.w + kBlock - 1) / kBlock, (P.h + kBlock - 1) / kBlock, bt.n), block(kBlock, kBlock);
    const int per_xcd = (grid.x * grid.y + 7) / 8;
    dim3 grid1(per_xcd * 8, bt.n);
    const int f = cost9 ? c2f_refine_split_factor(P.w, P.h, R, bt.n, no_split) : 0;
    launch_note(kLaunchRefine, P.w, P.h, bt.n, f, R);
    if (f) {
        dim3 gridf(per_xcd * f * 8, bt.n), gs((P.w + 63) / 64, (P.h + 3) / 4, bt.n), bs(64, 4);
        with_radius(R, [&](auto r) {
            if (f == 3) hipLaunchKernelGGL((k_c2f_refine_tiled<r(), 3>), gridf, block, 0, s, P, flow, lut, cost9, bt.stride);
            else hipLaunchKernelGGL((k_c2f_refine_tiled<r(), 4>), gridf, block, 0, s, P, flow, lut, cost9, bt.stride);
        });
        if (f == 3) hipLaunchKernelGGL(k_c2f_select<3>, gs, bs, 0, s, flow, cost9, P.w, P.h, bt.stride);
        else hipLaunchKernelGGL(k_c2f_select<4>, gs, bs, 0, s, flow, cost9, P.w, P.h, bt.stride);
        return;
    }
    if (!(R == 9 || R == 17) || !c2f_table_ok(P.w, P.h, R)) {
        hipLaunchKernelGGL(k_c2f_refine, grid, block, 0, s, P, flow, lut, R, bt.stride);
        return;
    }
    const bool window = (R == 9) ? EPPM_C2F_WINDOW : EPPM_C2F_WINDOW17;
    if (!window) with_radius(R, [&](auto r) { hipLaunchKernelGGL((k_c2f_refine_tiled<r(), 0>), grid1, block, 0, s, P, flow, lut, (float*)nullptr, bt.stride); });
    else if (R == 9) hipLaunchKernelGGL((k_c2f_refine_win<9>), grid1, dim3(kBlock, kBlock, 2), 0, s, P, flow, lut, bt.stride);
    else hipLaunchKernelGGL((k_c2f_refine_win4<17>), grid1, dim3(kBlock, kBlock, 4), 0, s, P, flow, lut, bt.stride);
}

}
```

eppm_amd/csrc/launchers_ref_abi.cpp:

```cpp
#include "stage_object.h"
#include "mblur.h"

using namespace eppm;

namespace {
struct DevState {
    float *lut_pm = nullptr, *lut_wmf = nullptr, *lut_blf = nullptr;
    int lut_R = -1;
    void* scratch[9] = {nullptr, nullptr, nullptr, nullptr, nullptr, nullptr, nullptr, nullptr, nullptr};
    size_t scratch_bytes[9] = {0, 0, 0, 0, 0, 0, 0, 0, 0};
    std::map<std::tuple<int, int, int, unsigned long long>, eppm_pm_rng*> rngs;
};
std::mutex g_mu;
std::map<int, DevState> g_dev;
hipStream_t g_stream = nullptr;
eppm_params g_prm = {9, 10, 30, 6, 10, 20, 1234ULL, 0, kNumLevels};
int g_launch_status = EPPM_OK;

int dev_state(DevState** out)
{
    int d = 0;
    HIPCHK(hipGetDevice(&d));
    DevState& s = g_dev[d];
    if (s.lut_R != g_prm.patch_r) {
// ... 311 lines not shown
    g_launch_status = mk_planes(ds, &P, d_img1, d_img2, d_census1, d_census2, w, h, img_pitch, census_pitch);
    if (g_launch_status != EPPM_OK) return;
    void* spec = nullptr;
    const size_t plane_bytes = cost_pitch * h;
    g_launch_status = get_scratch(ds, plane_bytes * 8, &spec, 4);
    if (g_launch_status != EPPM_OK) return;
    b.cache_plane = plane_bytes / 4;
    void* wl = nullptr;
    b.wl_units = pm_worklist_units(w, h, g_prm.seg_len);
    g_launch_status = get_scratch(ds, pm_worklist_words(w, h, g_prm.seg_len) * 4, &wl, 5);
    if (g_launch_status != EPPM_OK) return;
    b.p[0] = mk_problem(P, d_cost, (int16_t*)d_disp_vec, (int16_t*)tmp, r, 0, (float*)spec, (int32_t*)((char*)spec + plane_bytes * 4), sweep_list_on(opt_sweep_spec()) ? (uint32_t*)wl : nullptr);
    run_patchmatch(b, r, ds->lut_pm, g_prm, g_stream, opt_sweep_spec());
    if (b.p[0].nnf != (int16_t*)d_disp_vec && (g_launch_status = copy_d2d(d_disp_vec, b.p[0].nnf, disp_pitch * h)) != EPPM_OK) return;
    g_launch_status = finish();
}

extern "C" void baoCudaLeftRightCheck(eppm_short2* d_disp_vec, float* d_cost, eppm_short2* d_disp_vec2, float* d_cost2,
        int w, int h, size_t cost_pitch, size_t disp_pitch)
{
    std::lock_guard<std::mutex> lk(g_mu);
    launch_lr_check((int16_t*)d_disp_vec, d_cost, (const int16_t*)d_disp_vec2, w, h, (int)(cost_pitch / 4), (int)(disp_pitch / 4), g_stream);
    launch_lr_check((int16_t*)d_disp_vec2, d_cost2, (const int16_t*)d_disp_vec, w, h, (int)(cost_pitch / 4), (int)(disp_pitch / 4), g_stream);
    g_launch_status = finish();
}

extern "C" void baoCudaOutlierRemoval(eppm_short2* d_disp_vec, float* d_cost, int w, int h, size_t cost_pitch, size_t disp_pitch)
{
    LAUNCHER_BEGIN;
    void* tmp = nullptr;
    g_launch_status = get_scratch(ds, disp_pitch * h, &tmp);
    if (g_launch_status != EPPM_OK) return;
    if ((g_launch_status = copy_d2d(tmp, d_disp_vec, disp_pitch * h)) != EPPM_OK) return;
    launch_outlier((int16_t*)d_disp_vec, d_cost, (const int16_t*)tmp, w, h, (int)(cost_pitch / 4), (int)(disp_pitch / 4), g_stream);
    g_launch_status = finish();
}

extern "C" void baoCudaWeightedMedianFilter(eppm_short2* d_disp_vec, float* d_cost, eppm_uchar4* d_img, int w, int h,
        size_t img_pitch, size_t cost_pitch, size_t disp_pitch, int num_iter, bool is_only_occlusion)
{
    (void)d_cost; (void)cost_pitch;
    LAUNCHER_BEGIN;
    void* tmp = nullptr;
    g_launch_status = get_scratch(ds, disp_pitch * h, &tmp);
    if (g_launch_status != EPPM_OK) return;
    void* ws = nullptr;
    g_launch_status = get_scratch(ds, wmf_workspace_words(w, h, num_iter) * 4, &ws, 1);
    if (g_launch_status != EPPM_OK) return;
    int16_t* res = launch_wmf((int16_t*)d_disp_vec, (int16_t*)tmp, (const uint32_t*)d_img, (int)(img_pitch / 4), w, h, (int)(disp_pitch / 4),
                              ds->lut_wmf, num_iter, is_only_occlusion ? 1 : 0, (uint32_t*)ws, g_stream);
    if (res != (int16_t*)d_disp_vec && (g_launch_status = copy_d2d(d_disp_vec, res, disp_pitch * h)) != EPPM_OK) return;
    g_launch_status = finish();
}

extern "C" void baoCudaFillHole(eppm_short2* d_disp_vec, float* d_cost, eppm_uchar4* d_img, int w, int h,
        size_t img_pitch, size_t cost_pitch, size_t disp_pitch)
{
    (void)d_cost; (void)cost_pitch;
    LAUNCHER_BEGIN;
    void* tmp = nullptr;
    g_launch_status = get_scratch(ds, disp_pitch * h, &tmp);
    if (g_launch_status != EPPM_OK) return;
    if ((g_launch_status = copy_d2d(tmp, d_disp_vec, disp_pitch * h)) != EPPM_OK) return;
    launch_fill_holes((int16_t*)d_disp_vec, (const int16_t*)tmp, (const uint32_t*)d_img, (int)(img_pitch / 4), w, h, (int)(disp_pitch / 4), g_stream);
    g_launch_status = finish();
}

extern "C" void baoCudaNNF2Flow(eppm_float2* d_flow, eppm_short2* d_disp_vec, int w, int h, size_t disp_pitch, size_t flow_pitch)
{
    std::lock_guard<std::mutex> lk(g_mu);
    launch_nnf2flow((float*)d_flow, (int)(flow_pitch / 8), (const int16_t*)d_disp_vec, (int)(disp_pitch / 4), w, h, g_stream);
    g_launch_status = finish();
}

extern "C" void baoCudaBLFCostFilterRefine(eppm_float2* d_flow_vec, eppm_uchar4* d_img1, eppm_uchar4* d_img2, unsigned char* d_census1,
        unsigned char* d_census2, int w, int h, size_t img_pitch, size_t census_pitch)
{
    LAUNCHER_BEGIN;
    PlanesH P;
    g_launch_status = mk_planes(ds, &P, d_img1, d_img2, d_census1, d_census2, w, h, img_pitch, census_pitch);
    if (g_launch_status != EPPM_OK) return;
    float* cost9 = nullptr;
    if ((g_launch_status = split_scratch(ds, w, h, &cost9)) != EPPM_OK) return;
    launch_c2f_refine(P, (float*)d_flow_vec, ds->lut_pm, g_prm.patch_r, cost9, g_stream, kOnePair, opt_no_split() != 0);
    g_launch_status = finish();
}

extern "C" void baoCudaBLF_C2F(eppm_float2** pFlowPyr, eppm_uchar4** pImgPyr1, eppm_uchar4** pImgPyr2, unsigned char** pCensusPyr1,
        unsigned char** pCensusPyr2, eppm_float2** pTempPyr1, eppm_float2** pTempPyr2, int* arrH, int* arrW,
        size_t* arrPitchUchar4, size_t* arrPitchUchar1, int nLayerIdx)
{
    (void)pTempPyr1; (void)pTempPyr2;
    LAUNCHER_BEGIN;
    const int l = nLayerIdx;
    launch_resize_flow((float*)pFlowPyr[l], arrH[l], arrW[l], (const float*)pFlowPyr[l + 1], arrH[l + 1], arrW[l + 1], 2.0f, 1.0f, g_stream);
    launch_mul_scalar((float*)pFlowPyr[l], 2.0f, arrH[l], arrW[l], g_stream);
    PlanesH P;
    g_launch_status = mk_planes(ds, &P, pImgPyr1[l], pImgPyr2[l], pCensusPyr1[l], pCensusPyr2[l], arrW[l], arrH[l], arrPitchUchar4[l], arrPitchUchar1[l]);
    if (g_launch_status != EPPM_OK) return;
    float* cost9 = nullptr;
    if ((g_launch_status = split_scratch(ds, arrW[l], arrH[l], &cost9)) != EPPM_OK) return;
    launch_c2f_refine(P, (float*)pFlowPyr[l], ds->lut_pm, g_prm.patch_r, cost9, g_stream, kOnePair, opt_no_split() != 0);
    g_launch_status = finish();
}

#ifdef EPPM_TEST_HOOKS
extern "C" int eppm_test_c2f_refine_batch(float* d_flow, const uint32_t* d_img1, const uint32_t* d_img2, const uint8_t* d_census1,
        const uint8_t* d_census2, int w, int h, int npairs)
{
    if (!d_flow || !d_img1 || !d_img2 || !d_census1 || !d_census2 || w < 1 || h < 1 || npairs < 1)
        return set_err(EPPM_ERR_ARG, "eppm_test_c2f_refine_batch: bad argument");
    LAUNCHER_BEGIN_INT;
    const size_t n = (size_t)w * h, stride = n * 16;
    void *a = nullptr, *b = nullptr, *f = nullptr;
    CHK(get_scratch(ds, stride * npairs, &a, 2));
    CHK(get_scratch(ds, stride * npairs, &b, 3));
    CHK(get_scratch(ds, stride * npairs, &f, 0));
    for (int p = 0; p < npairs; p++) {
        launch_pack((char*)a + p * stride, w, d_img1 + p * n, w, d_census1 + p * n, w, w, h, g_stream);
        launch_pack((char*)b + p * stride, w, d_img2 + p * n, w, d_census2 + p * n, w, w, h, g_stream);
        CHK(copy_d2d((char*)f + p * stride, d_flow + p * n * 2, n * 8));
    }
    PlanesH P;
    P.pk1 = a; P.pk2 = b; P.w = w; P.h = h; P.pitch = w;
    launch_c2f_refine(P, (float*)f, ds->lut_pm, g_prm.patch_r, nullptr, g_stream, Batch{npairs, stride}, opt_no_split() != 0);
    for (int p = 0; p < npairs; p++) CHK(copy_d2d(d_flow + p * n * 2, (char*)f + p * stride, n * 8));
    return finish();
}
#endif

#ifdef EPPM_TEST_HOOKS
extern "C" int eppm_test_pm_search(eppm_pm_rng* r, float* d_cost, eppm_short2* d_nnf, const uint32_t* d_img1, const uint32_t* d_img2, int w, int h,
                                   int ndir, int npairs, int pretest, float* d_restw, float* d_pre_n, float* d_pre_d)
{
    if (!r || !d_cost || !d_nnf || !d_img1 || !d_img2 || w != r->w || h != r->h || ndir < 1 || ndir > 2 || npairs < 1)
        return set_err(EPPM_ERR_ARG, "eppm_test_pm_search: bad argument");
    LAUNCHER_BEGIN_INT;
    const int R = g_prm.patch_r;
    if (r->G != g_prm.num_guess || (R != 9 && R != 17)) return set_err(EPPM_ERR_ARG, "eppm_test_pm_search: num_guess %d / patch_r %d", r->G, R);
    const size_t n = (size_t)w * h;
    const int pad = (R + 2) & ~1, ppitch = parity_pitch(w, pad);
    size_t off = 0;
    auto carve = [&](size_t bytes) { const size_t o = off; off = (off + bytes + 255) & ~(size_t)255; return o; };
    size_t o_img[2], o_cen[2], o_pk[2], o_pc[2], o_pp[2], o_cost[2], o_nnf[2], o_rw[2], o_pn[2], o_pd[2];
    for (int k = 0; k < 2; k++) { o_img[k] = carve(n * 4); o_cen[k] = carve(n); o_pk[k] = carve(n * 16); o_pc[k] = carve(n * 4); o_pp[k] = carve((size_t)2 * h * ppitch * 4); }
    for (int k = 0; k < ndir; k++) { o_cost[k] = carve(n * 4); o_nnf[k] = carve(n * 4); o_rw[k] = carve(n * 4); o_pn[k] = carve(n * 4); o_pd[k] = carve(n * 4); }
    const size_t stride = (off + 4095) & ~(size_t)4095;
    void *slab = nullptr, *tab = nullptr;
    CHK(get_scratch(ds, stride * npairs, &slab, 0));
    CHK(get_scratch(ds, (size_t)r->gx * r->gy * 512 * r->G * sizeof(int16_t), &tab, 7));
    char* S = (char*)slab;
    for (int p = 0; p < npairs; p++) {
        CHK(copy_d2d(S + p * stride + o_img[0], d_img1 + p * n, n * 4));
        CHK(copy_d2d(S + p * stride + o_img[1], d_img2 + p * n, n * 4));
        for (int k = 0; k < ndir; k++) {
            CHK(copy_d2d(S + p * stride + o_cost[k], d_cost + (p * ndir + k) * n, n * 4));
            CHK(copy_d2d(S + p * stride + o_nnf[k], (const char*)d_nnf + (p * ndir + k) * n * 4, n * 4));
        }
    }
    const Batch bt{npairs, stride};
    CensusBatch cb;
    cb.n = 2;
    for (int k = 0; k < 2; k++) {
        CensusJob& J = cb.job[k];
        J.census = (uint8_t*)(S + o_cen[k]); J.cpitch = w; J.texels = S + o_pk[k]; J.tpitch = w; J.img = (const uint32_t*)(S + o_img[k]); J.ipitch = w;
        J.w = w; J.h = h; J.first_block = 0; J.packed = (uint32_t*)(S + o_pc[k]);
    }
    launch_census_batch(cb, g_stream, bt);
    for (int k = 0; k < 2; k++) launch_parity_planes((uint32_t*)(S + o_pp[k]), ppitch, pad, (const uint32_t*)(S + o_pc[k]), w, w, h, g_stream, bt);
    PmBatch b;
    b.n = ndir; b.cpitch = w; b.npitch = w; b.npairs = npairs; b.stride = stride;
    for (int k = 0; k < ndir; k++) {
        PlanesH P;
        P.pk1 = S + o_pk[k]; P.pk2 = S + o_pk[k ^ 1]; P.w = w; P.h = h; P.pitch = w;
        P.pc1 = (const uint32_t*)(S + o_pc[k]); P.pc2 = (const uint32_t*)(S + o_pc[k ^ 1]);
        P.pp1 = (const uint32_t*)(S + o_pp[k]); P.pp2 = (const uint32_t*)(S + o_pp[k ^ 1]); P.pp_pitch = ppitch; P.pp_pad = pad;
        b.p[k] = mk_problem(P, (float*)(S + o_cost[k]), (int16_t*)(S + o_nnf[k]), nullptr, nullptr, 0, nullptr, nullptr, nullptr, nullptr, (float*)(S + o_rw[k]));
    }
    PmRngDev d = r->dev();
    launch_pm_rand_table(d, r->work[0][r->cur[0]], (int16_t*)tab, r->G, g_stream);
    d.rand_tab = (const int16_t*)tab;
    if (pretest) {
        if (!pm_search_pretest_ready(b, d, R)) return set_err(EPPM_ERR_ARG, "eppm_test_pm_search: no two-phase search at patch_r %d", R);
        launch_pm_rest_weight(b, ds->lut_pm, R, g_stream);
        if (d_pre_n && d_pre_d) {
            PmPretestSums ps{};
            for (int k = 0; k < ndir; k++) { ps.n[k] = (float*)(S + o_pn[k]); ps.d[k] = (float*)(S + o_pd[k]); }
            launch_pm_pretest_probe(b, ds->lut_pm, R, ps, g_stream);
        }
    }
    launch_pm_random_search(b, d, ds->lut_pm, R, g_prm.search_range, g_prm.num_guess, g_stream, pretest != 0);
    for (int p = 0; p < npairs; p++)
        for (int k = 0; k < ndir; k++) {
            CHK(copy_d2d(d_cost + (p * ndir + k) * n, S + p * stride + o_cost[k], n * 4));
            CHK(copy_d2d((char*)d_nnf + (p * ndir + k) * n * 4, S + p * stride + o_nnf[k], n * 4));
            if (pretest && d_restw) CHK(copy_d2d(d_restw + (p * ndir + k) * n, S + p * stride + o_rw[k], n * 4));
            if (pretest && d_pre_n && d_pre_d) {
                CHK(copy_d2d(d_pre_n + (p * ndir + k) * n, S + p * stride + o_pn[k], n * 4));
                CHK(copy_d2d(d_pre_d + (p * ndir + k) * n, S + p * stride + o_pd[k], n * 4));
            }
        }
    return finish();
}
#endif

extern "C" void baoCudaFlowSmoothing(eppm_float2* d_flow, eppm_uchar4* d_img, int w, int h, size_t img_pitch, size_t flow_pitch)
{
    LAUNCHER_BEGIN;
    void* tmp = nullptr;
    g_launch_status = get_scratch(ds, flow_pitch * h, &tmp);
// ... 131 lines not shown
```

eppm_amd/csrc/pm_device.cuh:

```cuda
#pragma once
#include "eppm_device.cuh"

#ifndef EPPM_PARITY_SEARCH
#define EPPM_PARITY_SEARCH 1
#endif
#ifndef EPPM_PARITY_SPEC
#define EPPM_PARITY_SPEC 0
#endif
#ifndef EPPM_PARITY_COST
#define EPPM_PARITY_COST 1
#endif
#ifndef EPPM_COST_FIELD_TILE
#define EPPM_COST_FIELD_TILE 1
#endif
#ifndef EPPM_LPC9
#ifdef EPPM_TOL
#define EPPM_LPC9 32
#else
#define EPPM_LPC9 16
#endif
#endif
#ifndef EPPM_LPC17
#define EPPM_LPC17 64
#endif
// ... 110 lines not shown
__device__ __forceinline__ float patch_dist_any(const Planes& P, const PatchLut& L, int R, int x1, int y1, int x2, int y2) { return patch_dist(P, L, R, x1, y1, x2, y2); }
template <int M> __device__ __forceinline__ float patch_dist_any(const Planes&, const PatchLutT<M>&, int, int, int, int, int) { return 0.0f; }

#define EPPM_PM_PRAGMA_(x) _Pragma(#x)
#define EPPM_PM_UNROLL(n) EPPM_PM_PRAGMA_(unroll n)
template <int RT, int PK = 0, class LUT>
__device__ __forceinline__ float search_patch_dist(const Planes& P, const LUT& L, int R, const float4* __restrict__ s_src, int TW,
                                                   int tx, int ty, int x1, int y1, int x2, int y2, const PlanesH& PH)
{
    if (RT == 0) return patch_dist_any(P, L, R, x1, y1, x2, y2);
    constexpr int S = RT + 1;
    const int pitch16 = P.pitch << 4;
    const rgbf c1 = texel_rgb(s_src[(ty + RT) * TW + tx + RT]);
    const rgbf c2 = texel_rgb(texel_at(P.pk2, texel_off(pitch16, P.w, P.h, x2, y2)));
    PatchSum sum;
    constexpr int CS = tol_chunk(RT);
    static_assert(S % CS == 0, "whole chunks per row");
    if constexpr (PK == 2) {
        static_assert(S % 4 == 2, "a row = whole dwordx4 gathers + one dwordx2");
        const __amdgpu_buffer_rsrc_t rs = __builtin_amdgcn_make_buffer_rsrc(const_cast<uint32_t*>(PH.pp2), 0, 2 * P.h * PH.pp_pitch * 4, 0x00020000);
        const int xp = x2 - RT + PH.pp_pad;
        const int rb = ((xp & 1) * P.h) * PH.pp_pitch + (xp >> 1);
        uint32_t two = 2u;
        asm volatile("" : "+v"(two));
#pragma unroll 2
        for (int ii = 0; ii < S; ii++) {
            const int ro = (rb + iclamp(y2 + 2 * ii - RT, 0, P.h - 1) * PH.pp_pitch) * 4;
            const float4* __restrict__ srow = s_src + (ty + 2 * ii) * TW + tx;
            uint32_t wq[S];
#pragma unroll
            for (int g = 0; g < S / 4; g++) {
                const u32x4 v = __builtin_amdgcn_raw_buffer_load_b128(rs, ro + 16 * g, 0, 0);
                wq[4 * g] = v.x; wq[4 * g + 1] = v.y; wq[4 * g + 2] = v.z; wq[4 * g + 3] = v.w;
            }
            { const u32x2 v = __builtin_amdgcn_raw_buffer_load_b64(rs, ro + 4 * (S - 2), 0, 0); wq[S - 2] = v.x; wq[S - 1] = v.y; }
#ifdef EPPM_SEARCH_TERM_UNROLL
            constexpr int TU = EPPM_SEARCH_TERM_UNROLL;
#else
            constexpr int TU = (S % 5 == 0) ? 5 : (S % 9 == 0) ? 9 : S;
#endif
EPPM_PM_UNROLL((TU))
            for (int jj = 0; jj < S; jj++) {
                float ct, wt;
                patch_terms(srow[2 * jj], unpack_texel(wq[jj], two), c1, c2, L.gsp[ii * S + jj], L.tab(), ct, wt);
                sum.add(ct, wt);
                if ((jj + 1) % CS == 0) sum.flush();
            }
        }
        return sum.result();
    }
    const uint32_t* __restrict__ pc2 = PH.pc2;
    for (int ii = 0; ii < S; ii++) {
        const int i = 2 * ii - RT;
        const unsigned r2 = __umul24((unsigned)iclamp(y2 + i, 0, P.h - 1), (unsigned)pitch16);
        const float4* __restrict__ srow = s_src + (ty + 2 * ii) * TW + tx;
        for (int j0 = 0; j0 < S; j0 += 5) {
            float4 q1[5], q2[5];
            uint32_t w2[PK == 1 ? 5 : 1];
#pragma unroll
            for (int k = 0; k < 5; k++) {
                const int jj = min(j0 + k, S - 1);
                q1[k] = srow[2 * jj];
                const unsigned o2 = r2 + ((unsigned)iclamp(x2 + 2 * jj - RT, 0, P.w - 1) << 4);
                if (PK == 1) w2[k] = *reinterpret_cast<const uint32_t*>(reinterpret_cast<const char*>(pc2) + (o2 >> 2));
                else q2[k] = texel_at(P.pk2, o2);
            }
#pragma unroll
            for (int k = 0; k < 5; k++) {
                if (j0 + k < S) {
                    float ct, wt;
                    if (PK == 1) q2[k] = make_texel(w2[k], w2[k] >> 24);
                    patch_terms(q1[k], q2[k], c1, c2, L.gsp[ii * S + j0 + k], L.tab(), ct, wt);
                    sum.add(ct, wt);
                    if ((j0 + k + 1) % CS == 0) sum.flush();
                }
            }
        }
    }
    return sum.result();
}

constexpr int pre_row0(int S) { return (S - EPPM_SEARCH_PRE_ROWS) / 2; }
#ifndef EPPM_TOL
__device__ __forceinline__ float rest_weight_term(const rgbf c1, const float4 q1, float gsp)
{
    float a2 = max_abs_diff(c1, texel_rgb(q1));
    a2 *= a2;
    return fast_exp(div_ad2(-a2)) * gsp;
}
template <int RT, class LUT>
__device__ __forceinline__ void search_patch_centre_rows(const Planes& P, const LUT& L, const float4* __restrict__ s_src, int TW, int tx, int ty,
                                                         int x2, int y2, const PlanesH& PH, float& cs, float& ws)
{
    constexpr int S = RT + 1, I0 = pre_row0(S);
    static_assert(S % 4 == 2 && EPPM_SEARCH_PRE_ROWS >= 1 && EPPM_SEARCH_PRE_ROWS <= S, "rows of whole dwordx4 gathers + one dwordx2");
    const int pitch16 = P.pitch << 4;
    const rgbf c1 = texel_rgb(s_src[(ty + RT) * TW + tx + RT]);
    const rgbf c2 = texel_rgb(texel_at(P.pk2, texel_off(pitch16, P.w, P.h, x2, y2)));
    const __amdgpu_buffer_rsrc_t rs = __builtin_amdgcn_make_buffer_rsrc(const_cast<uint32_t*>(PH.pp2), 0, 2 * P.h * PH.pp_pitch * 4, 0x00020000);
    const int xp = x2 - RT + PH.pp_pad;
    const int rb = ((xp & 1) * P.h) * PH.pp_pitch + (xp >> 1);
    cs = 0.0f; ws = 0.0f;
#pragma unroll 2
    for (int ii = I0; ii < I0 + EPPM_SEARCH_PRE_ROWS; ii++) {
        const int ro = (rb + iclamp(y2 + 2 * ii - RT, 0, P.h - 1) * PH.pp_pitch) * 4;
        const float4* __restrict__ srow = s_src + (ty + 2 * ii) * TW + tx;
        uint32_t wq[S];
#pragma unroll
        for (int g = 0; g < S / 4; g++) {
            const u32x4 v = __builtin_amdgcn_raw_buffer_load_b128(rs, ro + 16 * g, 0, 0);
            wq[4 * g] = v.x; wq[4 * g + 1] = v.y; wq[4 * g + 2] = v.z; wq[4 * g + 3] = v.w;
        }
        { const u32x2 v = __builtin_amdgcn_raw_buffer_load_b64(rs, ro + 4 * (S - 2), 0, 0); wq[S - 2] = v.x; wq[S - 1] = v.y; }
EPPM_PM_UNROLL(((S % 5 == 0) ? 5 : S))
        for (int jj = 0; jj < S; jj++) {
            float ct, wt;
            patch_terms(srow[2 * jj], unpack_texel(wq[jj], 0u), c1, c2, L.gsp[ii * S + jj], L.tab(), ct, wt);
            patch_accum(cs, ws, ct, wt);
        }
    }
}
#endif

template <int RT>
__device__ __forceinline__ void pm_stage_tile(float4* __restrict__ s_src, const Planes& P, int bx, int by, int tid)
{
    constexpr int TW = kBlock + 2 * RT;
    const int x0 = bx * kBlock - RT, y0 = by * kBlock - RT;
    for (int t = tid; t < TW * TW; t += 256) {
        const int sy = iclamp(y0 + t / TW, 0, P.h - 1), sx = iclamp(x0 + t % TW, 0, P.w - 1);
        s_src[t] = P.pk1[(unsigned)(sy * P.pitch + sx)];
    }
}

static inline bool pm_parity_adopted(int R, bool exact_adopts)
{
#ifdef EPPM_TOL
    (void)exact_adopts;
    return R == 9 || R == 17;
#else
    return exact_adopts && R == 9;
#endif
}
static inline bool pm_has_parity(const PmBatch& b, int R, bool exact_adopts)
{
    return pm_parity_adopted(R, exact_adopts) && b.p[0].P.pp2 && (b.n < 2 || b.p[1].P.pp2);
}

template <int LPC>
__device__ __forceinline__ float dpp_prev_lane(float v)
{
    if (LPC == 4) return __int_as_float(__builtin_amdgcn_update_dpp(0, __float_as_int(v), 0x93 , 0xf, 0xf, false));
    if (LPC == 16) return __int_as_float(__builtin_amdgcn_update_dpp(0, __float_as_int(v), 0x121 , 0xf, 0xf, false));
    return __int_as_float(__builtin_amdgcn_update_dpp(0, __float_as_int(v), 0x138 , 0xf, 0xf, false));
}

template <int R, int LPC>
__host__ __device__ constexpr int coop_chunk()
{
#ifdef EPPM_TOL
    return tol_chunk(R);
#else
    return ((R + 1) * (R + 1) + LPC - 1) / LPC;
#endif
}
template <int LPC, int CH, int NS, int NL>
__device__ __forceinline__ void coop_chain_sum(const float (&tc)[CH], const float (&tw)[CH], float& ac, float& aw)
{
#ifdef EPPM_TOL
    float pc = 0.0f, pw = 0.0f;
#pragma unroll
    for (int q = 0; q < CH; q++) patch_accum(pc, pw, tc[q], tw[q]);
// ... 62 lines not shown
```

eppm_amd/stages.py:

```python
import ctypes as C

import numpy as np

from ._lib import CParams, check, check_launcher, lib, probe_dispatch
from .api import float2, short2, uchar4


class Dev:

    def __init__(self, arr=None, shape=None, dtype=None, pitched=False):
        if arr is not None:
            arr = np.ascontiguousarray(arr)
            shape, dtype = arr.shape, arr.dtype
        self.h, self.w = shape
        self.dtype = np.dtype(dtype)
        row = self.w * self.dtype.itemsize
        self.ptr = C.c_void_p()
        if pitched:
            pitch = C.c_size_t()
            check(lib().eppm_malloc_pitched(C.byref(self.ptr), C.byref(pitch), C.c_size_t(row), C.c_size_t(self.h)), "malloc_pitched")
            self.pitch = pitch.value
        else:
            check(lib().eppm_malloc_device(C.byref(self.ptr), C.c_size_t(row * self.h)), "malloc")
            self.pitch = row
# ... 196 lines not shown
    check(lib().eppm_probe_search_pretest(iteration, w, h, patch_r, problems, npairs, out, C.byref(eps)), "eppm_probe_search_pretest")
    return bool(out[0]), out[1], out[2], out[3], eps.value, bool(out[4])


def patchmatch(P):
    n, c = Dev(shape=(P.h, P.w), dtype=short2), Dev(shape=(P.h, P.w), dtype=np.float32)
    lib().baoCudaPatchMatch(n.ptr, c.ptr, *P.args(), P.w, P.h, _sz(P.i1.pitch), _sz(c.pitch), _sz(n.pitch), _sz(P.c1.pitch))
    check_launcher("baoCudaPatchMatch")
    return n.get(), c.get()


def left_right_check(nnf1, cost1, nnf2, cost2):
    h, w = nnf1.shape
    a, b, c, d = Dev(nnf1), Dev(cost1), Dev(nnf2), Dev(cost2)
    lib().baoCudaLeftRightCheck(a.ptr, b.ptr, c.ptr, d.ptr, w, h, _sz(b.pitch), _sz(a.pitch))
    check_launcher("baoCudaLeftRightCheck")
    return a.get(), b.get(), c.get(), d.get()


def outlier_removal(nnf, cost):
    h, w = nnf.shape
    a, b = Dev(nnf), Dev(cost)
    lib().baoCudaOutlierRemoval(a.ptr, b.ptr, w, h, _sz(b.pitch), _sz(a.pitch))
    check_launcher("baoCudaOutlierRemoval")
    return a.get(), b.get()


def weighted_median(nnf, img, num_iter=20, only_occlusion=True):
    h, w = nnf.shape
    a, i = Dev(nnf), Dev(img, pitched=True)
    lib().baoCudaWeightedMedianFilter(a.ptr, None, i.ptr, w, h, _sz(i.pitch), _sz(w * 4), _sz(a.pitch), num_iter, C.c_bool(only_occlusion))
    check_launcher("baoCudaWeightedMedianFilter")
    return a.get()


def fill_holes(nnf, img):
    h, w = nnf.shape
    a, i = Dev(nnf), Dev(img, pitched=True)
    lib().baoCudaFillHole(a.ptr, None, i.ptr, w, h, _sz(i.pitch), _sz(w * 4), _sz(a.pitch))
    check_launcher("baoCudaFillHole")
    return a.get()


def nnf2flow(nnf):
    h, w = nnf.shape
    a, f = Dev(nnf), Dev(shape=(h, w), dtype=float2)
    lib().baoCudaNNF2Flow(f.ptr, a.ptr, w, h, _sz(a.pitch), _sz(f.pitch))
    check_launcher("baoCudaNNF2Flow")
    return f.get()


def resize_flow(flow, out_h, out_w, ratio=2.0):
    h, w = flow.shape
    a, b = Dev(flow), Dev(shape=(out_h, out_w), dtype=float2)
    check(lib().eppm_resize_flow(b.ptr, out_h, out_w, a.ptr, h, w, C.c_float(ratio)), "resize_flow")
    return b.get()


def flow_upsample(coarse, img):
    h, w = img.shape
    hc, wc = coarse.shape
    a, i, b = Dev(coarse), Dev(img, pitched=True), Dev(shape=(h, w), dtype=float2)
    check(lib().eppm_flow_upsample(b.ptr, h, w, a.ptr, hc, wc, i.ptr, _sz(i.pitch)), "eppm_flow_upsample")
    return b.get()


def c2f_refine(flow, P):
    f = Dev(flow)
    lib().baoCudaBLFCostFilterRefine(f.ptr, *P.args(), P.w, P.h, _sz(P.i1.pitch), _sz(P.c1.pitch))
    check_launcher("baoCudaBLFCostFilterRefine")
    return f.get()


def c2f_refine_batch(flows, planes):
    n = len(flows)
    h, w = flows[0].shape
    f = Dev(np.concatenate([np.ascontiguousarray(x, float2) for x in flows]))
    i1, i2, c1, c2 = (Dev(np.concatenate([np.ascontiguousarray(p[k]) for p in planes])) for k in range(4))
    check(lib().eppm_test_c2f_refine_batch(f.ptr, i1.ptr, i2.ptr, c1.ptr, c2.ptr, w, h, n), "eppm_test_c2f_refine_batch")
    out = f.get()
    return [out[k * h:(k + 1) * h] for k in range(n)]


def blf_c2f(flow_coarse, P_fine, coarse_dims):
    ch, cw = coarse_dims
    fine = Dev(shape=(P_fine.h, P_fine.w), dtype=float2)
    coarse = Dev(flow_coarse)
    tab = lambda a, b: (C.c_void_p * 2)(a, b)
    arrH = (C.c_int * 2)(P_fine.h, ch)
    arrW = (C.c_int * 2)(P_fine.w, cw)
    p4 = (C.c_size_t * 2)(P_fine.i1.pitch, 0)
    pc = (C.c_size_t * 2)(P_fine.c1.pitch, 0)
    lib().baoCudaBLF_C2F(tab(fine.ptr, coarse.ptr), tab(P_fine.i1.ptr, None), tab(P_fine.i2.ptr, None), tab(P_fine.c1.ptr, None),
                         tab(P_fine.c2.ptr, None), None, None, arrH, arrW, p4, pc, 0)
    check_launcher("baoCudaBLF_C2F")
    return fine.get()


def flow_smoothing(flow, img):
    h, w = flow.shape
    f, i = Dev(flow), Dev(img, pitched=True)
    lib().baoCudaFlowSmoothing(f.ptr, i.ptr, w, h, _sz(i.pitch), _sz(f.pitch))
    check_launcher("baoCudaFlowSmoothing")
    return f.get()


def temporal_prior(prev, backward=False):
    d_prev = Dev(np.ascontiguousarray(prev, short2))
    d_out = Dev(shape=prev.shape, dtype=short2)
    check(lib().eppm_temporal_prior(d_out.ptr, d_prev.ptr, d_prev.h, d_prev.w, int(bool(backward))), "eppm_temporal_prior")
    check(lib().eppm_device_synchronize(), "eppm_device_synchronize")
    return d_out.get()


def temporal_prior_batch(prevs, backward=False, armed=None, calls=1):
    prevs = np.ascontiguousarray(prevs, short2)
    n, h, w = prevs.shape
    d_prev = Dev(prevs.reshape(n * h, w))
    d_out = Dev(shape=(n * h, w), dtype=short2)
    flags = None if armed is None else (C.c_uint8 * n)(*[int(bool(x)) for x in armed])
    out = []
    for _ in range(calls):
        check(lib().eppm_temporal_prior_batch(d_out.ptr, d_prev.ptr, h, w, int(bool(backward)), n, flags), "eppm_temporal_prior_batch")
        check(lib().eppm_device_synchronize(), "eppm_device_synchronize")
        out.append(d_out.get().reshape(n, h, w))
    return out[0] if calls == 1 else out


def flow_to_color(flow, max_disp_x=20.0, max_disp_y=20.0):
    h, w = flow.shape
    f, c = Dev(flow), Dev(shape=(h, w), dtype=uchar4)
    check(lib().eppm_flow_to_color(c.ptr, f.ptr, h, w, C.c_float(max_disp_x), C.c_float(max_disp_y)), "eppm_flow_to_color")
    return c.get()
```

Measured before the change: 238.1 Mflow-vectors/s.

## Add two-phase pretest to window coarse-to-fine refine to skip full candidate costs

The R=9 window refine kernel now first evaluates the 9 candidates on a few central patch rows, picks the best candidate, computes its full cost, then uses a bound (partial numerator against best cost times partial denominator plus the rest-weight sum) to decide which other candidates need full evaluation. Candidates that provably lose are skipped, cutting the per-pixel cost work. Survivors are compacted into per-block lists stored in the tile padding. The change adds shared-memory atomics, extra barriers and register pressure, and falls back to the full path when denominators are tiny.

```diff
diff --git a/eppm_amd/_lib.py b/eppm_amd/_lib.py
--- a/eppm_amd/_lib.py
+++ b/eppm_amd/_lib.py
@@ -156,7 +156,7 @@
 ]
 
 
-TEST_SYMBOLS = ["eppm_test_set_option", "eppm_test_c2f_refine_batch", "eppm_probe_c2f_window", "eppm_probe_dispatch", "eppm_probe_fast_exp", "eppm_probe_div_const", "eppm_probe_delta_table",
+TEST_SYMBOLS = ["eppm_test_set_option", "eppm_test_c2f_refine_batch", "eppm_test_c2f_refine_pre", "eppm_test_c2f_refine_probe", "eppm_probe_c2f_pretest", "eppm_probe_c2f_window", "eppm_probe_dispatch", "eppm_probe_fast_exp", "eppm_probe_div_const", "eppm_probe_delta_table",
                 "eppm_probe_unpack_texel", "eppm_probe_pm_parity", "eppm_probe_ctx_rng_states", "eppm_test_pm_search", "eppm_probe_search_pretest", "eppm_probe_launch_log"]
 
 _variant = None
diff --git a/eppm_amd/csrc/api_internal.h b/eppm_amd/csrc/api_internal.h
--- a/eppm_amd/csrc/api_internal.h
+++ b/eppm_amd/csrc/api_internal.h
@@ -61,6 +61,8 @@
 static inline int opt_no_split() { return g_opt_no_split.load(); }
 static inline int opt_force_split() { return g_opt_force_split.load(); }
 static inline int opt_search_pre() { return g_opt_search_pre.load(); }
+EPPM_HIDDEN extern std::atomic<int> g_opt_c2f_pre;
+static inline int opt_c2f_pre() { return g_opt_c2f_pre.load(); }
 EPPM_HIDDEN extern std::atomic<int> g_opt_alloc_fill;
 static inline int opt_alloc_fill() { return g_opt_alloc_fill.load(); }
 EPPM_HIDDEN hipError_t alloc_fill(hipError_t e, void* p, size_t bytes, bool pinned);
@@ -70,6 +72,7 @@
 static constexpr int opt_no_split() { return 0; }
 static constexpr int opt_force_split() { return 0; }
 static constexpr int opt_search_pre() { return -1; }
+static constexpr int opt_c2f_pre() { return -1; }
 static constexpr int opt_alloc_fill() { return -1; }
 #endif
 
diff --git a/eppm_amd/csrc/c2f_device.cuh b/eppm_amd/csrc/c2f_device.cuh
--- a/eppm_amd/csrc/c2f_device.cuh
+++ b/eppm_amd/csrc/c2f_device.cuh
@@ -24,6 +24,17 @@
 #ifndef EPPM_C2F_WIN_WAVES
 #define EPPM_C2F_WIN_WAVES 4
 #endif
+#ifndef EPPM_C2F_PRE
+#define EPPM_C2F_PRE 1
+#endif
+#ifndef EPPM_C2F_PRE_ROWS
+#define EPPM_C2F_PRE_ROWS 5
+#endif
+#ifndef EPPM_C2F_PRE_EPS
+#define EPPM_C2F_PRE_EPS 0x1p-13f
+#endif
+#define EPPM_C2F_PRE_DMIN 0x1p-60f
+#define EPPM_C2F_PRE_RHSMIN 0x1p-100f
 #ifndef EPPM_C2F_SPLIT_BELOW_WAVES
 #define EPPM_C2F_SPLIT_BELOW_WAVES 1024
 #endif
@@ -101,6 +112,10 @@
 }
 
 template <int R> struct C2fSrcTile { static constexpr int TWU = kBlock + 2 * R, TW = (TWU + 15) / 16 * 16; };
+template <int R> struct C2fPreList {
+    static constexpr int PADB = (C2fSrcTile<R>::TW - C2fSrcTile<R>::TWU) * 16, KROWS = PADB ? (256 * 8 + PADB - 1) / PADB : 0;
+    static constexpr int CAP = PADB ? (C2fSrcTile<R>::TWU - KROWS) * (PADB / 2) : 0;
+};
 struct C2fOff { int dx16, up; };
 
 template <int R>
@@ -338,4 +353,62 @@
     for (int n = 0; n < 3; n++) { outA[n] = cs[n] / ws[n]; outB[n] = cs[3 + n] / ws[3 + n]; }
 }
 
-}
+#ifndef EPPM_TOL
+template <int R, int PA, int PB, int WW, int I0, int I1, int NC>
+__device__ __forceinline__ void c2f_rows2_win(const PatchLutT<R + 1>& L, const float4* __restrict__ s_src, int TW, int tx, int ty,
+                                              const rgbf c1, const rgbf (&c2)[NC], const float4* __restrict__ s_win, int wbase,
+                                              float (&cs)[2 * NC], float (&ws)[2 * NC])
+{
+    constexpr int S = R + 1;
+    constexpr int TA = (PA == 0) ? 0 : PA - 1, TB = (PB == 0) ? 0 : PB - 1;
+    const C2fTables<R>& T = c2f_tables<R>();
+    const rgbf c1w = c2f_weight_centre(c1);
+    rgbf c2w[2 * NC];
+#pragma unroll
+    for (int n = 0; n < NC; n++) { c2w[n] = c2f_weight_centre(c2[n]); c2w[NC + n] = c2w[n]; }
+#pragma unroll
+    for (int n = 0; n < 2 * NC; n++) { cs[n] = 0.0f; ws[n] = 0.0f; }
+#pragma unroll 1
+    for (int ii = I0; ii < I1; ii++) {
+        const int rdyA = (PA == 0) ? 2 * ii - R : T.rowdy[TA][ii];
+        const int rdyB = (PB == 0) ? 2 * ii - R : T.rowdy[TB][ii];
+EPPM_UNROLL(EPPM_C2F_UNROLL)
+        for (int jj = 0; jj < S; jj++) {
+            const C2fSample smp = c2f_sample(L, c1w, s_src[(ty + 2 * ii) * TW + tx + 2 * jj], ii * S + jj);
+            const int soffA = (rdyA + ((PA != 0) ? T.off[TA][ii * S + jj].up : 0)) * (WW * 16) + ((PA == 0) ? (2 * jj - R) * 16 : T.off[TA][ii * S + jj].dx16);
+            const int soffB = (rdyB + ((PB != 0) ? T.off[TB][ii * S + jj].up : 0)) * (WW * 16) + ((PB == 0) ? (2 * jj - R) * 16 : T.off[TB][ii * S + jj].dx16);
+            const char* wa = reinterpret_cast<const char*>(s_win) + (wbase + soffA);
+            const char* wb = reinterpret_cast<const char*>(s_win) + (wbase + soffB);
+            float4 q[2 * NC];
+#pragma unroll
+            for (int n = 0; n < NC; n++) { q[n] = *reinterpret_cast<const float4*>(wa + n * (WW * 16)); q[NC + n] = *reinterpret_cast<const float4*>(wb + n * (WW * 16)); }
+            c2f_terms<2 * NC>(L, smp, c2w, q, cs, ws);
+        }
+    }
+}
+
+template <int R, int PASS, int WW>
+__device__ __forceinline__ float c2f_one_win(const PatchLutT<R + 1>& L, const float4* __restrict__ s_src, int TW, int tx, int ty,
+                                             const rgbf c1, const rgbf c2, const float4* __restrict__ s_win, int wbase)
+{
+    constexpr int S = R + 1;
+    constexpr int TP = (PASS == 0) ? 0 : PASS - 1;
+    const C2fTables<R>& T = c2f_tables<R>();
+    const rgbf c1w = c2f_weight_centre(c1), c2w[1] = {c2f_weight_centre(c2)};
+    float cs[1] = {0.0f}, ws[1] = {0.0f};
+#pragma unroll 1
+    for (int ii = 0; ii < S; ii++) {
+        const int rdy = (PASS == 0) ? 2 * ii - R : T.rowdy[TP][ii];
+EPPM_UNROLL(EPPM_C2F_UNROLL)
+        for (int jj = 0; jj < S; jj++) {
+            const C2fSample smp = c2f_sample(L, c1w, s_src[(ty + 2 * ii) * TW + tx + 2 * jj], ii * S + jj);
+            const int soff = (rdy + ((PASS != 0) ? T.off[TP][ii * S + jj].up : 0)) * (WW * 16) + ((PASS == 0) ? (2 * jj - R) * 16 : T.off[TP][ii * S + jj].dx16);
+            const float4 q[1] = {*reinterpret_cast<const float4*>(reinterpret_cast<const char*>(s_win) + (wbase + soff))};
+            c2f_terms<1>(L, smp, c2w, q, cs, ws);
+        }
+    }
+    return cs[0] / ws[0];
+}
+#endif
+
+}
diff --git a/eppm_amd/csrc/context.cpp b/eppm_amd/csrc/context.cpp
--- a/eppm_amd/csrc/context.cpp
+++ b/eppm_amd/csrc/context.cpp
@@ -117,7 +117,7 @@
     HIPCHK(hipSetDevice(device));
     eppm_ctx* c = new eppm_ctx();
     c->device = device; c->prm = p; c->h = h; c->w = w; c->npairs = npairs; c->n_active = 1;
-    c->opt_sweep_spec = opt_sweep_spec(); c->opt_no_split = opt_no_split(); c->opt_search_pre = opt_search_pre();
+    c->opt_sweep_spec = opt_sweep_spec(); c->opt_no_split = opt_no_split(); c->opt_search_pre = opt_search_pre(); c->opt_c2f_pre = opt_c2f_pre();
     c->nl = pyr_init_dim(c->H, c->W, h, w, p.levels, 0.5f);
     const int L = c->nl - 1;
     if (c->H[L] < 1 || c->W[L] < 1 || (c->W[L] + p.seg_len - 1) / p.seg_len > 1024 || (c->H[L] + p.seg_len - 1) / p.seg_len > 1024) {
diff --git a/eppm_amd/csrc/context.h b/eppm_amd/csrc/context.h
--- a/eppm_amd/csrc/context.h
+++ b/eppm_amd/csrc/context.h
@@ -10,7 +10,7 @@
     int device = 0;
     hipStream_t stream = nullptr;
     bool own_stream = false;
-    int opt_sweep_spec = -1, opt_no_split = 0, opt_search_pre = -1;
+    int opt_sweep_spec = -1, opt_no_split = 0, opt_search_pre = -1, opt_c2f_pre = -1;
     eppm_params prm;
     int h = 0, w = 0, nl = 0;
     int stop_level = 0;
diff --git a/eppm_amd/csrc/ctx_compute.cpp b/eppm_amd/csrc/ctx_compute.cpp
--- a/eppm_amd/csrc/ctx_compute.cpp
+++ b/eppm_amd/csrc/ctx_compute.cpp
@@ -113,7 +113,7 @@
         launch_resize_flow(d.a[l], c->H[l], c->W[l], r, c->H[l + 1], c->W[l + 1], 2.0f, 2.0f, s, bt);
         stage_end(c, c->ev);
         stage_begin(c, c->ev, level_stage.s[kStageRefine][d.bwd][l], d.dominant);
-        launch_c2f_refine(planes(c, l, d.swap), d.a[l], c->lut_pm, c->prm.patch_r, c->c2f_cost9[l], s, bt, c->opt_no_split != 0);
+        launch_c2f_refine(planes(c, l, d.swap), d.a[l], c->lut_pm, c->prm.patch_r, c->c2f_cost9[l], s, bt, c->opt_no_split != 0, c->opt_c2f_pre);
         stage_end(c, c->ev, d.dominant);
         stage_begin(c, c->ev, level_stage.s[kStageBlf][d.bwd][l]);
         blf(d.b[l], d.a[l], l);
diff --git a/eppm_amd/csrc/eppm_device.cuh b/eppm_amd/csrc/eppm_device.cuh
--- a/eppm_amd/csrc/eppm_device.cuh
+++ b/eppm_amd/csrc/eppm_device.cuh
@@ -156,6 +156,14 @@
     for (int t = tid; t < kDeltaSlots; t += nthreads) D.t2[t] = src[256 + t];
 }
 __device__ __forceinline__ rgbf texel_rgb(const float4 t) { return rgbf{t.x, t.y, t.z}; }
+#ifndef EPPM_TOL
+__device__ __forceinline__ float rest_weight_term(const rgbf c1, const float4 q1, float gsp)
+{
+    float a2 = max_abs_diff(c1, texel_rgb(q1));
+    a2 *= a2;
+    return fast_exp(div_ad2(-a2)) * gsp;
+}
+#endif
 
 __device__ __forceinline__ float4 tex_px(const float4* img, int pitch, int w, int h, int x, int y)
 {
diff --git a/eppm_amd/csrc/eppm_internal.h b/eppm_amd/csrc/eppm_internal.h
--- a/eppm_amd/csrc/eppm_internal.h
+++ b/eppm_amd/csrc/eppm_internal.h
@@ -161,7 +161,9 @@
 EPPM_DECISION int c2f_refine_split_factor(int w, int h, int R, int npairs = 1, bool no_split = false);
 bool c2f_refine_wants_split(int w, int h, int R, int npairs = 1, bool no_split = false);
 bool c2f_window_span(int R, int* span_x, int* span_y);
-void launch_c2f_refine(const PlanesH& P, float* flow, const float* lut, int R, float* cost9, hipStream_t s, Batch bt = kOnePair, bool no_split = false);
+void launch_c2f_refine(const PlanesH& P, float* flow, const float* lut, int R, float* cost9, hipStream_t s, Batch bt = kOnePair, bool no_split = false,
+                       int pre = -1, unsigned* stat = nullptr, float* probe = nullptr);
+void c2f_pretest_knobs(int R, int* on, int* row0, int* rows, int* cap, float* eps, float* dmin, float* rhsmin);
 void launch_flow_blf(float* out, const float* in, const uint32_t* img, int ipitch, int w, int h, int flow_pitch,
                      const float* blf_lut, hipStream_t s, Batch bt = kOnePair);
 EPPM_DECISION int flow_blf_pixels_per_lane(int w, int h, int npairs = 1);
diff --git a/eppm_amd/csrc/k_c2f_refine.hip b/eppm_amd/csrc/k_c2f_refine.hip
--- a/eppm_amd/csrc/k_c2f_refine.hip
+++ b/eppm_amd/csrc/k_c2f_refine.hip
@@ -112,9 +112,10 @@
     flow[(y * P.w + x) * 2 + 1] = (float)(by - y);
 }
 
-template <int R>
+template <int R, bool PROBE = false>
 __global__ __launch_bounds__(512) __attribute__((amdgpu_waves_per_eu(EPPM_C2F_WIN_WAVES, EPPM_C2F_WIN_WAVES)))
-void k_c2f_refine_win(PlanesH Ph, float* __restrict__ flow_, const float* __restrict__ lut, size_t pstride)
+void k_c2f_refine_win(PlanesH Ph, float* __restrict__ flow_, const float* __restrict__ lut, size_t pstride, int pre, unsigned* __restrict__ stat,
+                      float* __restrict__ probe)
 {
     using W = C2fWinShape<R>;
     constexpr int TWU = C2fSrcTile<R>::TWU, TW = C2fSrcTile<R>::TW, WW = W::WW, WH = W::WH;
@@ -123,6 +124,9 @@
     __shared__ float4 s_src[TWU * TW];
     __shared__ float4 s_win[WH * WW];
     __shared__ int s_mm[4];
+#ifndef EPPM_TOL
+    __shared__ int s_pre[8];
+#endif
     float* __restrict__ flow = pair_ptr(flow_, pstride, blockIdx.y);
     const int ptid = threadIdx.y * kBlock + threadIdx.x;
     const int grp = threadIdx.z;
@@ -134,6 +138,9 @@
     int x0, y0, part;
     if (!c2f_tile_origin<0>(P, x0, y0, part)) return;
     if (tid == 0) { s_mm[0] = 0x7fffffff; s_mm[1] = -0x7fffffff; s_mm[2] = 0x7fffffff; s_mm[3] = -0x7fffffff; }
+#ifndef EPPM_TOL
+    if (tid < 8) s_pre[tid] = 0;
+#endif
     for (int t = tid; t < TWU * TWU; t += 512) {
         const int ry = t / TWU, rx = t % TWU;
         const int sy = iclamp(y0 + ry - R, 0, P.h - 1), sx = iclamp(x0 + rx - R, 0, P.w - 1);
@@ -161,6 +168,159 @@
         }
     }
     __syncthreads();
+#ifndef EPPM_TOL
+    int path = 3;
+    if (pre && coherent && mxx >= mnx) {
+        constexpr int S = R + 1, I0 = (S - EPPM_C2F_PRE_ROWS) / 2, I1 = I0 + EPPM_C2F_PRE_ROWS;
+        constexpr int PADB = C2fPreList<R>::PADB, KROWS = C2fPreList<R>::KROWS, CAP = C2fPreList<R>::CAP;
+        static_assert(PADB % 8 == 0 && PADB > 0 && KROWS < TWU, "keys and items do not straddle a row's padding");
+        auto pad = [&](int o) -> char* { return reinterpret_cast<char*>(s_src) + (o / PADB) * (TW * 16) + TWU * 16 + (o % PADB); };
+        auto key_at = [&](int p) -> unsigned long long* { return reinterpret_cast<unsigned long long*>(pad(p * 8)); };
+        auto item_at = [&](int i) -> uint16_t* { return reinterpret_cast<uint16_t*>(pad(KROWS * PADB + i * 2)); };
+        const int lane = tid & 63;
+        float N[18], D[18], U = 0.0f;
+        unsigned vmask = 0;
+        rgbf c1 = {0.0f, 0.0f, 0.0f};
+        if (known) {
+            c1 = texel_rgb(s_src[(threadIdx.y + R) * TW + threadIdx.x + R]);
+#pragma unroll 1
+            for (int ii = 0; ii < S; ii++) {
+                if (ii >= I0 && ii < I1) continue;
+                const float4* __restrict__ srow = s_src + (threadIdx.y + 2 * ii) * TW + threadIdx.x;
+#pragma unroll
+                for (int jj = 0; jj < S; jj++) U += rest_weight_term(c1, srow[2 * jj], L.gsp[ii * S + jj]);
+            }
+        }
+#pragma unroll
+        for (int m = 0; m < 3; m++) {
+            const int cx = (int)(int16_t)(ccx + m - 1);
+            float cs[6] = {0.0f, 0.0f, 0.0f, 0.0f, 0.0f, 0.0f}, ws[6] = {0.0f, 0.0f, 0.0f, 0.0f, 0.0f, 0.0f};
+            if (known && !(cx < 0 || cx >= P.w)) {
+                const int wbase = ((ccy - 1 - wy0) * WW + (cx - wx0)) * 16;
+                rgbf c2[3];
+#pragma unroll
+                for (int n = 0; n < 3; n++) {
+                    c2[n] = texel_rgb(*reinterpret_cast<const float4*>(reinterpret_cast<const char*>(s_win) + wbase + n * (WW * 16)));
+                    const int cy = (int)(int16_t)(ccy + n - 1);
+                    if (!(cy < 0 || cy >= P.h)) vmask |= 1u << (m * 3 + n);
+                }
+                if (grp == 0) c2f_rows2_win<R, 3, 2, WW, I0, I1, 3>(L, s_src, TW, threadIdx.x, threadIdx.y, c1, c2, s_win, wbase, cs, ws);
+                else c2f_rows2_win<R, 1, 0, WW, I0, I1, 3>(L, s_src, TW, threadIdx.x, threadIdx.y, c1, c2, s_win, wbase, cs, ws);
+            }
+#pragma unroll
+            for (int n = 0; n < 3; n++) { N[m * 3 + n] = cs[n]; D[m * 3 + n] = ws[n]; N[9 + m * 3 + n] = cs[3 + n]; D[9 + m * 3 + n] = ws[3 + n]; }
+        }
+        if (PROBE && known) {
+            float* __restrict__ pp = probe + ((size_t)blockIdx.y * P.h * P.w + (size_t)y * P.w + x) * 73;
+            const int qa = (grp == 0 ? 3 : 1) * 9, qb = (grp == 0 ? 2 : 0) * 9;
+#pragma unroll
+            for (int k = 0; k < 9; k++) { pp[qa + k] = N[k]; pp[36 + qa + k] = D[k]; pp[qb + k] = N[9 + k]; pp[36 + qb + k] = D[9 + k]; }
+            if (grp == 1) pp[72] = U;
+        }
+        bool small = false;
+#pragma unroll
+        for (int k = 0; k < 9; k++)
+            if ((vmask >> k) & 1) small = small || !(D[k] > EPPM_C2F_PRE_DMIN) || !(D[9 + k] > EPPM_C2F_PRE_DMIN);
+        if (small) s_pre[0] = 1;
+        if (grp == 1) {
+            int ks = 15;
+            float e_best = 0.0f;
+#pragma unroll
+            for (int k = 0; k < 9; k++) {
+                if (!((vmask >> k) & 1)) continue;
+                const float e = c2f_min(N[k] / D[k], N[9 + k] / D[9 + k]);
+                if (ks == 15 || e < e_best) { e_best = e; ks = k; }
+            }
+            *key_at(ptid) = 0xfffffffffffffff0ull | (unsigned)ks;
+        }
+        __syncthreads();
+        path = 1;
+        if (!s_pre[0]) {
+            const int ks = (int)(*reinterpret_cast<const uint32_t*>(key_at(ptid)) & 15u);
+            const bool live = known && ks != 15;
+            if (live) {
+                const int cx = (int)(int16_t)(ccx + ks / 3 - 1);
+                const int wbase = ((ccy - 1 + ks % 3 - wy0) * WW + (cx - wx0)) * 16;
+                const rgbf c2[1] = {texel_rgb(*reinterpret_cast<const float4*>(reinterpret_cast<const char*>(s_win) + wbase))};
+                float cs[2], ws[2];
+                if (grp == 0) c2f_rows2_win<R, 3, 2, WW, 0, S, 1>(L, s_src, TW, threadIdx.x, threadIdx.y, c1, c2, s_win, wbase, cs, ws);
+                else c2f_rows2_win<R, 1, 0, WW, 0, S, 1>(L, s_src, TW, threadIdx.x, threadIdx.y, c1, c2, s_win, wbase, cs, ws);
+                const float c = c2f_min(cs[0] / ws[0], cs[1] / ws[1]);
+                atomicMin(key_at(ptid), ((unsigned long long)__float_as_uint(c) << 4) | (unsigned)ks);
+            }
+            __syncthreads();
+            unsigned sa = 0, sb = 0, tested = 0;
+            if (live) {
+                const float B = __uint_as_float((uint32_t)(*key_at(ptid) >> 4));
+#pragma unroll
+                for (int k = 0; k < 9; k++) {
+                    if (!((vmask >> k) & 1) || k == ks) continue;
+                    const float ra = B * (D[k] + U), rb = B * (D[9 + k] + U);
+                    if (!(N[k] * (1.0f - EPPM_C2F_PRE_EPS) >= ra && ra >= EPPM_C2F_PRE_RHSMIN)) sa |= 1u << k;
+                    if (!(N[9 + k] * (1.0f - EPPM_C2F_PRE_EPS) >= rb && rb >= EPPM_C2F_PRE_RHSMIN)) sb |= 1u << k;
+                    tested += 2;
+                }
+            }
+            const int na = __popc(sa), nb = __popc(sb);
+            int ia = na, ib = nb;
+#pragma unroll
+            for (int d = 1; d < 64; d <<= 1) {
+                const int ta = __shfl_up(ia, d), tb = __shfl_up(ib, d);
+                if (lane >= d) { ia += ta; ib += tb; }
+            }
+            const int pa = grp == 0 ? 3 : 1, pb = grp == 0 ? 2 : 0;
+            int wa = 0, wb = 0;
+            if (lane == 63) { wa = atomicAdd(&s_pre[1 + pa], ia); wb = atomicAdd(&s_pre[1 + pb], ib); }
+            wa = __shfl(wa, 63); wb = __shfl(wb, 63);
+            if (stat && tested) { atomicAdd(stat + 4, tested); atomicAdd(stat + 5, tested - (unsigned)(na + nb)); }
+            __syncthreads();
+            int cnt[4], chb[5];
+            chb[0] = 0;
+#pragma unroll
+            for (int p = 0; p < 4; p++) { cnt[p] = s_pre[1 + p]; chb[p + 1] = chb[p] + ((cnt[p] + 63) >> 6); }
+            path = 2;
+            if (chb[4] * 64 <= CAP) {
+                path = 0;
+                {
+                    int at = chb[pa] * 64 + wa + ia - na;
+                    for (unsigned s = sa; s; s &= s - 1) *item_at(at++) = (uint16_t)(ptid | ((__ffs(s) - 1) << 8));
+                    at = chb[pb] * 64 + wb + ib - nb;
+                    for (unsigned s = sb; s; s &= s - 1) *item_at(at++) = (uint16_t)(ptid | ((__ffs(s) - 1) << 8));
+                }
+                __syncthreads();
+                for (int c = tid >> 6; c < chb[4]; c += 8) {
+                    const int p = __builtin_amdgcn_readfirstlane((c >= chb[1]) + (c >= chb[2]) + (c >= chb[3]));
+                    const int idx = (c - chb[p]) * 64 + lane;
+                    if (idx < cnt[p]) {
+                        const unsigned it = *item_at(chb[p] * 64 + idx);
+                        const int ip = it & 255, k = it >> 8, tx = ip & (kBlock - 1), ty = ip / kBlock;
+                        const int px = x0 + tx, py = y0 + ty;
+                        const int qcx = c2f_centre(flow[(py * P.w + px) * 2], px), qcy = c2f_centre(flow[(py * P.w + px) * 2 + 1], py);
+                        const int cx = (int)(int16_t)(qcx + k / 3 - 1);
+                        const int wbase = ((qcy - 1 + k % 3 - wy0) * WW + (cx - wx0)) * 16;
+                        const rgbf q1 = texel_rgb(s_src[(ty + R) * TW + tx + R]);
+                        const rgbf q2 = texel_rgb(*reinterpret_cast<const float4*>(reinterpret_cast<const char*>(s_win) + wbase));
+                        float c_;
+                        if (p == 3) c_ = c2f_one_win<R, 3, WW>(L, s_src, TW, tx, ty, q1, q2, s_win, wbase);
+                        else if (p == 2) c_ = c2f_one_win<R, 2, WW>(L, s_src, TW, tx, ty, q1, q2, s_win, wbase);
+                        else if (p == 1) c_ = c2f_one_win<R, 1, WW>(L, s_src, TW, tx, ty, q1, q2, s_win, wbase);
+                        else c_ = c2f_one_win<R, 0, WW>(L, s_src, TW, tx, ty, q1, q2, s_win, wbase);
+                        atomicMin(key_at(ip), ((unsigned long long)__float_as_uint(c_) << 4) | (unsigned)k);
+                    }
+                }
+                __syncthreads();
+                if (stat && tid == 0) atomicAdd(stat + 0, 1u);
+                if (grp != 1 || !inimg) return;
+                if (!known) { c2f_store_flow(flow, y * P.w + x, 0, 0); return; }
+                int k = (int)(*key_at(ptid) & 15u);
+                if (k == 15) k = 4;
+                c2f_store_flow(flow, y * P.w + x, (int)(int16_t)(ccx + k / 3 - 1) - x, (int)(int16_t)(ccy + k % 3 - 1) - y);
+                return;
+            }
+        }
+    }
+    if (stat && tid == 0) atomicAdd(stat + path, 1u);
+#endif
     float res[9];
     float res1[9];
     if (known) {
@@ -379,6 +539,18 @@
     return true;
 }
 
+void c2f_pretest_knobs(int R, int* on, int* row0, int* rows, int* cap, float* eps, float* dmin, float* rhsmin)
+{
+#ifdef EPPM_TOL
+    *on = 0;
+#else
+    *on = EPPM_C2F_PRE;
+#endif
+    *row0 = (R + 1 - EPPM_C2F_PRE_ROWS) / 2; *rows = EPPM_C2F_PRE_ROWS;
+    *cap = C2fPreList<9>::CAP;
+    *eps = EPPM_C2F_PRE_EPS; *dmin = EPPM_C2F_PRE_DMIN; *rhsmin = EPPM_C2F_PRE_RHSMIN;
+}
+
 static bool c2f_table_ok(int w, int h, int R) { return (w + R < 32764) && (h + R < 32764); }
 
 int c2f_refine_split_factor(int w, int h, int R, int npairs, bool no_split)
@@ -398,7 +570,8 @@
     else f(std::integral_constant<int, 17>{});
 }
 
-void launch_c2f_refine(const PlanesH& P, float* flow, const float* lut, int R, float* cost9, hipStream_t s, Batch bt, bool no_split)
+void launch_c2f_refine(const PlanesH& P, float* flow, const float* lut, int R, float* cost9, hipStream_t s, Batch bt, bool no_split, int pre,
+                       unsigned* stat, float* probe)
 {
     dim3 grid((P.w + kBlock - 1) / kBlock, (P.h + kBlock - 1) / kBlock, bt.n), block(kBlock, kBlock);
     const int per_xcd = (grid.x * grid.y + 7) / 8;
@@ -421,7 +594,8 @@
     }
     const bool window = (R == 9) ? EPPM_C2F_WINDOW : EPPM_C2F_WINDOW17;
     if (!window) with_radius(R, [&](auto r) { hipLaunchKernelGGL((k_c2f_refine_tiled<r(), 0>), grid1, block, 0, s, P, flow, lut, (float*)nullptr, bt.stride); });
-    else if (R == 9) hipLaunchKernelGGL((k_c2f_refine_win<9>), grid1, dim3(kBlock, kBlock, 2), 0, s, P, flow, lut, bt.stride);
+    else if (R == 9 && probe) hipLaunchKernelGGL((k_c2f_refine_win<9, true>), grid1, dim3(kBlock, kBlock, 2), 0, s, P, flow, lut, bt.stride, 1, stat, probe);
+    else if (R == 9) hipLaunchKernelGGL((k_c2f_refine_win<9>), grid1, dim3(kBlock, kBlock, 2), 0, s, P, flow, lut, bt.stride, pre < 0 ? EPPM_C2F_PRE : pre, stat, (float*)nullptr);
     else hipLaunchKernelGGL((k_c2f_refine_win4<17>), grid1, dim3(kBlock, kBlock, 4), 0, s, P, flow, lut, bt.stride);
 }
 
diff --git a/eppm_amd/csrc/launchers_ref_abi.cpp b/eppm_amd/csrc/launchers_ref_abi.cpp
--- a/eppm_amd/csrc/launchers_ref_abi.cpp
+++ b/eppm_amd/csrc/launchers_ref_abi.cpp
@@ -417,7 +417,7 @@
     if (g_launch_status != EPPM_OK) return;
     float* cost9 = nullptr;
     if ((g_launch_status = split_scratch(ds, w, h, &cost9)) != EPPM_OK) return;
-    launch_c2f_refine(P, (float*)d_flow_vec, ds->lut_pm, g_prm.patch_r, cost9, g_stream, kOnePair, opt_no_split() != 0);
+    launch_c2f_refine(P, (float*)d_flow_vec, ds->lut_pm, g_prm.patch_r, cost9, g_stream, kOnePair, opt_no_split() != 0, opt_c2f_pre());
     g_launch_status = finish();
 }
 
@@ -435,22 +435,29 @@
     if (g_launch_status != EPPM_OK) return;
     float* cost9 = nullptr;
     if ((g_launch_status = split_scratch(ds, arrW[l], arrH[l], &cost9)) != EPPM_OK) return;
-    launch_c2f_refine(P, (float*)pFlowPyr[l], ds->lut_pm, g_prm.patch_r, cost9, g_stream, kOnePair, opt_no_split() != 0);
+    launch_c2f_refine(P, (float*)pFlowPyr[l], ds->lut_pm, g_prm.patch_r, cost9, g_stream, kOnePair, opt_no_split() != 0, opt_c2f_pre());
     g_launch_status = finish();
 }
 
 #ifdef EPPM_TEST_HOOKS
-extern "C" int eppm_test_c2f_refine_batch(float* d_flow, const uint32_t* d_img1, const uint32_t* d_img2, const uint8_t* d_census1,
-        const uint8_t* d_census2, int w, int h, int npairs)
-{
+static int c2f_refine_batch(float* d_flow, const uint32_t* d_img1, const uint32_t* d_img2, const uint8_t* d_census1,
+        const uint8_t* d_census2, int w, int h, int npairs, int pre, unsigned* stat, float* d_probe = nullptr)
+{
+#ifdef EPPM_TOL
+    if (pre == 1 || d_probe) return set_err(EPPM_ERR_ARG, "the tolerance library's window refine has no two-phase form");
+#endif
     if (!d_flow || !d_img1 || !d_img2 || !d_census1 || !d_census2 || w < 1 || h < 1 || npairs < 1)
         return set_err(EPPM_ERR_ARG, "eppm_test_c2f_refine_batch: bad argument");
     LAUNCHER_BEGIN_INT;
     const size_t n = (size_t)w * h, stride = n * 16;
-    void *a = nullptr, *b = nullptr, *f = nullptr;
+    void *a = nullptr, *b = nullptr, *f = nullptr, *st = nullptr;
     CHK(get_scratch(ds, stride * npairs, &a, 2));
     CHK(get_scratch(ds, stride * npairs, &b, 3));
-    CHK(get_scratch(ds, stride * npairs, &f, 0));
+    CHK(get_scratch(ds, stride * npairs + 32, &f, 0));
+    if (stat) {
+        st = (char*)f + stride * npairs;
+        HIPCHK(hipMemsetAsync(st, 0, 32, g_stream));
+    }
     for (int p = 0; p < npairs; p++) {
         launch_pack((char*)a + p * stride, w, d_img1 + p * n, w, d_census1 + p * n, w, w, h, g_stream);
         launch_pack((char*)b + p * stride, w, d_img2 + p * n, w, d_census2 + p * n, w, w, h, g_stream);
@@ -458,9 +465,28 @@
     }
     PlanesH P;
     P.pk1 = a; P.pk2 = b; P.w = w; P.h = h; P.pitch = w;
-    launch_c2f_refine(P, (float*)f, ds->lut_pm, g_prm.patch_r, nullptr, g_stream, Batch{npairs, stride}, opt_no_split() != 0);
+    if (d_probe) HIPCHK(hipMemsetAsync(d_probe, 0xff, n * npairs * 73 * 4, g_stream));
+    launch_c2f_refine(P, (float*)f, ds->lut_pm, g_prm.patch_r, nullptr, g_stream, Batch{npairs, stride}, opt_no_split() != 0, pre, (unsigned*)st, d_probe);
     for (int p = 0; p < npairs; p++) CHK(copy_d2d(d_flow + p * n * 2, (char*)f + p * stride, n * 8));
-    return finish();
+    if (stat) { HIPCHK(hipMemcpyAsync(stat, st, 32, hipMemcpyDeviceToHost, g_stream)); HIPCHK(hipStreamSynchronize(g_stream)); }
+    return finish();
+}
+extern "C" int eppm_test_c2f_refine_batch(float* d_flow, const uint32_t* d_img1, const uint32_t* d_img2, const uint8_t* d_census1,
+        const uint8_t* d_census2, int w, int h, int npairs)
+{
+    return c2f_refine_batch(d_flow, d_img1, d_img2, d_census1, d_census2, w, h, npairs, opt_c2f_pre(), nullptr);
+}
+extern "C" int eppm_test_c2f_refine_pre(float* d_flow, const uint32_t* d_img1, const uint32_t* d_img2, const uint8_t* d_census1,
+        const uint8_t* d_census2, int w, int h, int npairs, int pre, unsigned* stat)
+{
+    if (!stat || pre < -1 || pre > 1) return set_err(EPPM_ERR_ARG, "eppm_test_c2f_refine_pre: bad argument");
+    return c2f_refine_batch(d_flow, d_img1, d_img2, d_census1, d_census2, w, h, npairs, pre, stat);
+}
+extern "C" int eppm_test_c2f_refine_probe(float* d_flow, const uint32_t* d_img1, const uint32_t* d_img2, const uint8_t* d_census1,
+        const uint8_t* d_census2, int w, int h, int npairs, float* d_probe)
+{
+    if (!d_probe || g_prm.patch_r != 9) return set_err(EPPM_ERR_ARG, "eppm_test_c2f_refine_probe: bad argument (patch radius 9 only)");
+    return c2f_refine_batch(d_flow, d_img1, d_img2, d_census1, d_census2, w, h, npairs, 1, nullptr, d_probe);
 }
 #endif
 
diff --git a/eppm_amd/csrc/pm_device.cuh b/eppm_amd/csrc/pm_device.cuh
--- a/eppm_amd/csrc/pm_device.cuh
+++ b/eppm_amd/csrc/pm_device.cuh
@@ -216,12 +216,6 @@
 
 constexpr int pre_row0(int S) { return (S - EPPM_SEARCH_PRE_ROWS) / 2; }
 #ifndef EPPM_TOL
-__device__ __forceinline__ float rest_weight_term(const rgbf c1, const float4 q1, float gsp)
-{
-    float a2 = max_abs_diff(c1, texel_rgb(q1));
-    a2 *= a2;
-    return fast_exp(div_ad2(-a2)) * gsp;
-}
 template <int RT, class LUT>
 __device__ __forceinline__ void search_patch_centre_rows(const Planes& P, const LUT& L, const float4* __restrict__ s_src, int TW, int tx, int ty,
                                                          int x2, int y2, const PlanesH& PH, float& cs, float& ws)
diff --git a/eppm_amd/stages.py b/eppm_amd/stages.py
--- a/eppm_amd/stages.py
+++ b/eppm_amd/stages.py
@@ -302,6 +302,35 @@
     return [out[k * h:(k + 1) * h] for k in range(n)]
 
 
+def c2f_refine_pre(flows, planes, pre):
+    n = len(flows)
+    h, w = flows[0].shape
+    f = Dev(np.concatenate([np.ascontiguousarray(x, float2) for x in flows]))
+    i1, i2, c1, c2 = (Dev(np.concatenate([np.ascontiguousarray(p[k]) for p in planes])) for k in range(4))
+    stat = (C.c_uint * 8)()
+    check(lib().eppm_test_c2f_refine_pre(f.ptr, i1.ptr, i2.ptr, c1.ptr, c2.ptr, w, h, n, int(pre), stat), "eppm_test_c2f_refine_pre")
+    out = f.get()
+    return [out[k * h:(k + 1) * h] for k in range(n)], tuple(stat[:6])
+
+
+def c2f_refine_probe(flows, planes):
+    n = len(flows)
+    h, w = flows[0].shape
+    f = Dev(np.concatenate([np.ascontiguousarray(x, float2) for x in flows]))
+    i1, i2, c1, c2 = (Dev(np.concatenate([np.ascontiguousarray(p[k]) for p in planes])) for k in range(4))
+    pr = Dev(shape=(n * h, w * 73), dtype=np.float32)
+    check(lib().eppm_test_c2f_refine_probe(f.ptr, i1.ptr, i2.ptr, c1.ptr, c2.ptr, w, h, n, pr.ptr), "eppm_test_c2f_refine_probe")
+    out, p = f.get(), pr.get().reshape(n, h, w, 73)
+    return [out[k * h:(k + 1) * h] for k in range(n)], p[..., :36].reshape(n, h, w, 4, 9), p[..., 36:72].reshape(n, h, w, 4, 9), p[..., 72]
+
+
+def probe_c2f_pretest(patch_r=9):
+    out = (C.c_int * 4)()
+    fl = (C.c_float * 3)()
+    check(lib().eppm_probe_c2f_pretest(patch_r, out, fl), "eppm_probe_c2f_pretest")
+    return bool(out[0]), out[1], out[2], out[3], fl[0], fl[1], fl[2]
+
+
 def blf_c2f(flow_coarse, P_fine, coarse_dims):
     ch, cw = coarse_dims
     fine = Dev(shape=(P_fine.h, P_fine.w), dtype=float2)
```

Result: faster. 254.0 Mflow-vectors/s (median of 6 runs) (+6.7%).
